# eth-cscs/conflux

Hardware: AMD Instinct MI355X
Metric: fp64_lu_tflops (higher is better)
Workload: dtype f64; 1 GPU; conflux LU N=16384 v=512 grid 1x1x1 (BASELINE cfg for 1 GPU); N=16384, v=512, grid=1x1x1

## Files before the change

conflux_amd/__init__.py:

```python
import ctypes
import os

_HERE = os.path.dirname(os.path.abspath(__file__))
_LIB_PATH = os.path.join(_HERE, "libconflux_lu.so")

UID_BYTES = 128


class ConfluxLuError(RuntimeError):
    pass


def _load():
    if not os.path.exists(_LIB_PATH):
        raise ConfluxLuError(
            f"HIP engine not built: {_LIB_PATH} missing. "
            "Run `make -C conflux_amd` (or __graft_entry__.build()). "
            "The product has no CPU fallback.")
    lib = ctypes.CDLL(_LIB_PATH)
    lib.conflux_lu_create.argtypes = [ctypes.c_int] * 7 + [
        ctypes.c_char_p, ctypes.POINTER(ctypes.c_void_p)]
    lib.conflux_lu_make_uid.argtypes = [ctypes.c_char_p]
    lib.conflux_lu_init_matrix.argtypes = [ctypes.c_void_p, ctypes.c_uint64]
    lib.conflux_lu_init_matrix_spd.argtypes = [ctypes.c_void_p, ctypes.c_uint64]
    lib.conflux_chol_factor.argtypes = [ctypes.c_void_p,
                                        ctypes.POINTER(ctypes.c_double)]
    lib.conflux_lu_set_matrix_local.argtypes = [ctypes.c_void_p, ctypes.c_void_p]
    lib.conflux_lu_set_matrix_sim.argtypes = [ctypes.c_void_p, ctypes.c_int,
                                              ctypes.c_void_p]
    lib.conflux_lu_store_factors.argtypes = [ctypes.c_void_p, ctypes.c_int]
    lib.conflux_lu_set_pivoting.argtypes = [ctypes.c_void_p, ctypes.c_int]
    lib.conflux_lu_factor.argtypes = [ctypes.c_void_p,
                                      ctypes.POINTER(ctypes.c_double)]
    lib.conflux_lu_get_factors.argtypes = [ctypes.c_void_p, ctypes.c_void_p,
                                           ctypes.c_void_p]
    lib.conflux_lu_get_factors_sim.argtypes = [ctypes.c_void_p, ctypes.c_int,
                                               ctypes.c_void_p, ctypes.c_void_p]
    lib.conflux_lu_dims.argtypes = [ctypes.c_void_p] + [
        ctypes.POINTER(ctypes.c_int)] * 6
    lib.conflux_lu_kernel_stats.argtypes = [
        ctypes.c_void_p, ctypes.c_int, ctypes.POINTER(ctypes.c_double),
        ctypes.POINTER(ctypes.c_long), ctypes.POINTER(ctypes.c_double)]
    lib.conflux_lu_validate.argtypes = [ctypes.c_void_p,
                                        ctypes.POINTER(ctypes.c_double)]
    lib.conflux_chol_validate.argtypes = [ctypes.c_void_p,
                                          ctypes.POINTER(ctypes.c_double)]
    lib.conflux_lu_destroy.argtypes = [ctypes.c_void_p]
    lib.conflux_lu_build_info.restype = ctypes.c_char_p
    lib.conflux_lu_debug_dgemm.argtypes = [
        ctypes.c_int, ctypes.c_longlong, ctypes.c_int, ctypes.c_void_p,
        ctypes.c_void_p, ctypes.c_void_p]
    lib.conflux_lu_debug_getrf.argtypes = [ctypes.c_int, ctypes.c_int,
                                           ctypes.c_void_p, ctypes.c_void_p]
    lib.conflux_lu_debug_set_panel_glue.argtypes = [ctypes.c_int]
    lib.conflux_lu_debug_set_panel_reg.argtypes = [ctypes.c_int]
    lib.conflux_lu_debug_set_panel_publish.argtypes = [ctypes.c_int]
    lib.conflux_lu_debug_set_panel_phase_stats.argtypes = [ctypes.c_int]
    lib.conflux_lu_debug_panel_phase_stats.argtypes = [ctypes.c_void_p]
    lib.conflux_lu_debug_set_trsm_stripe.argtypes = [ctypes.c_int]
    lib.conflux_lu_debug_trsm_stripe_width.argtypes = []
    lib.conflux_lu_debug_trsm_ld.argtypes = [
        ctypes.c_int, ctypes.c_int, ctypes.c_int, ctypes.c_longlong,
        ctypes.c_longlong, ctypes.c_longlong, ctypes.c_void_p,
        ctypes.c_void_p]
    lib.conflux_lu_debug_dgemm_bench.argtypes = [
        ctypes.c_int, ctypes.c_longlong, ctypes.c_int, ctypes.c_int,
        ctypes.POINTER(ctypes.c_double)]
    lib.conflux_lu_debug_trsm.argtypes = [
        ctypes.c_int, ctypes.c_int, ctypes.c_longlong, ctypes.c_int,
        ctypes.c_void_p, ctypes.c_void_p]
    lib.conflux_lu_solve.argtypes = [
        ctypes.c_void_p, ctypes.c_void_p, ctypes.c_int,
        ctypes.POINTER(ctypes.c_double)]
    lib.conflux_chol_solve.argtypes = lib.conflux_lu_solve.argtypes
    lib.conflux_lu_debug_trsm_left.argtypes = [
        ctypes.c_int, ctypes.c_int, ctypes.c_int, ctypes.c_longlong,
        ctypes.c_longlong, ctypes.c_void_p, ctypes.c_void_p]
    lib.conflux_lu_debug_update_skinny.argtypes = [
        ctypes.c_int, ctypes.c_int, ctypes.c_int, ctypes.c_longlong,
        ctypes.c_void_p, ctypes.c_void_p, ctypes.c_void_p]
    lib.conflux_lu_solve_refined.argtypes = [
        ctypes.c_void_p, ctypes.c_void_p, ctypes.c_int, ctypes.c_int,
        ctypes.c_void_p, ctypes.c_void_p, ctypes.POINTER(ctypes.c_int),
        ctypes.POINTER(ctypes.c_double)]
    lib.conflux_chol_solve_refined.argtypes = \
        lib.conflux_lu_solve_refined.argtypes
    lib.conflux_lu_debug_residual_dd.argtypes = [
        ctypes.c_int, ctypes.c_int, ctypes.c_int, ctypes.c_longlong,
        ctypes.c_void_p, ctypes.c_void_p, ctypes.c_void_p, ctypes.c_void_p]
    lib.conflux_lu_debug_residual_group_width.argtypes = []
    lib.conflux_lu_debug_residual_dd_bench.argtypes = [
        ctypes.c_int, ctypes.c_int, ctypes.c_int, ctypes.c_int,
        ctypes.POINTER(ctypes.c_double), ctypes.POINTER(ctypes.c_double)]
    lib.conflux_lu_solve_trans.argtypes = lib.conflux_lu_solve.argtypes
    lib.conflux_lu_rcond.argtypes = [
        ctypes.c_void_p, ctypes.c_int, ctypes.POINTER(ctypes.c_double),
        ctypes.POINTER(ctypes.c_double), ctypes.POINTER(ctypes.c_int),
        ctypes.POINTER(ctypes.c_double)]
    lib.conflux_chol_rcond.argtypes = [
        ctypes.c_void_p, ctypes.POINTER(ctypes.c_double),
        ctypes.POINTER(ctypes.c_double), ctypes.POINTER(ctypes.c_int),
        ctypes.POINTER(ctypes.c_double)]
    lib.conflux_lu_debug_trsm_left_trans.argtypes = \
        lib.conflux_lu_debug_trsm_left.argtypes
    lib.conflux_lu_debug_update_skinny_t.argtypes = \
        lib.conflux_lu_debug_update_skinny.argtypes
    return lib


_lib = None


def lib():
    global _lib
    if _lib is None:
        _lib = _load()
    return _lib


def _chk(rc, what):
    if rc != 0:
        raise ConfluxLuError(f"{what} failed: rc={rc}")


class Engine:

    def __init__(self, N, v, Px, Py, Pz, rank=-1, world=None, uid=None):
        import numpy as np
        self.N, self.v, self.Px, self.Py, self.Pz = N, v, Px, Py, Pz
        P = Px * Py * Pz
        world = P if world is None else world
        self.world = world
        self.sim = rank < 0
        self._h = ctypes.c_void_p()
        _chk(lib().conflux_lu_create(N, v, Px, Py, Pz, rank, world, uid,
                                     ctypes.byref(self._h)), "create")
        d = [ctypes.c_int() for _ in range(6)]
        _chk(lib().conflux_lu_dims(self._h, *[ctypes.byref(x) for x in d]),
             "dims")
        self.Ml, self.Nl, self.Nt, self.nlayr, self.M, self.Npad = \
            (x.value for x in d)

    @staticmethod
    def make_uid():
        buf = ctypes.create_string_buffer(UID_BYTES)
        _chk(lib().conflux_lu_make_uid(buf), "make_uid")
        return buf.raw

    def init_matrix(self, seed=42):
        _chk(lib().conflux_lu_init_matrix(self._h, seed), "init_matrix")

    def set_matrix_global(self, A):
        import numpy as np
        assert self.sim
        v = self.v
        for pi in range(self.Px):
            for pj in range(self.Py):
                loc = np.zeros((self.Ml, self.Nl))
                for lti in range(self.Ml // v):
                    for ltj in range(self.Nl // v):
                        gti, gtj = lti * self.Px + pi, ltj * self.Py + pj
                        loc[lti * v:(lti + 1) * v, ltj * v:(ltj + 1) * v] = \
                            A[gti * v:(gti + 1) * v, gtj * v:(gtj + 1) * v]
                loc = np.ascontiguousarray(loc)
                for pk in range(self.Pz):
                    g = (pi * self.Py + pj) * self.Pz + pk
                    buf = loc if pk == 0 else None
                    _chk(lib().conflux_lu_set_matrix_sim(
                        self._h, g,
                        buf.ctypes.data_as(ctypes.c_void_p) if buf is not None
                        else None), "set_matrix_sim")

    def set_matrix_local(self, local):
        ptr = None
        if local is not None:
            import numpy as np
            local = np.ascontiguousarray(local, dtype=np.float64)
            ptr = local.ctypes.data_as(ctypes.c_void_p)
        _chk(lib().conflux_lu_set_matrix_local(self._h, ptr), "set_matrix")

    def store_factors(self, enable):
        _chk(lib().conflux_lu_store_factors(self._h, int(enable)), "store")

    def set_pivoting(self, mode):
        _chk(lib().conflux_lu_set_pivoting(self._h, int(mode)), "pivoting")

    def factor(self):
        ms = ctypes.c_double()
        _chk(lib().conflux_lu_factor(self._h, ctypes.byref(ms)), "factor")
        return ms.value

    def init_matrix_spd(self, seed=42):
        _chk(lib().conflux_lu_init_matrix_spd(self._h, seed), "init_spd")

    def factor_cholesky(self):
        ms = ctypes.c_double()
        _chk(lib().conflux_chol_factor(self._h, ctypes.byref(ms)), "chol")
        return ms.value

    def validate(self):
        r = ctypes.c_double()
        _chk(lib().conflux_lu_validate(self._h, ctypes.byref(r)), "validate")
        return r.value

    def validate_cholesky(self):
        r = ctypes.c_double()
        _chk(lib().conflux_chol_validate(self._h, ctypes.byref(r)),
             "chol_validate")
        return r.value

    def _solve(self, fn, what, B, return_ms):
        import numpy as np
        B = np.asarray(B)
        if B.ndim not in (1, 2) or B.shape[0] != self.Npad:
            raise ValueError(
                f"{what}: B must be ({self.Npad},) or ({self.Npad}, nrhs), "
                f"got {B.shape}")
        X = np.array(B, dtype=np.float64, order="C")
        nrhs = 1 if X.ndim == 1 else X.shape[1]
        ms = ctypes.c_double()
        _chk(fn(self._h, X.ctypes.data_as(ctypes.c_void_p), nrhs,
                ctypes.byref(ms)), what)
        return (X, ms.value) if return_ms else X

    def solve(self, B, return_ms=False):
        return self._solve(lib().conflux_lu_solve, "solve", B, return_ms)

    def solve_cholesky(self, B, return_ms=False):
        return self._solve(lib().conflux_chol_solve, "solve_cholesky", B,
                           return_ms)

    def solve_transposed(self, B, return_ms=False):
        return self._solve(lib().conflux_lu_solve_trans, "solve_transposed",
                           B, return_ms)

    def _rcond(self, what, call, return_info):
        rc = ctypes.c_double()
        an = ctypes.c_double()
        ns = ctypes.c_int()
        ms = ctypes.c_double()
        _chk(call(ctypes.byref(rc), ctypes.byref(an), ctypes.byref(ns),
                  ctypes.byref(ms)), what)
        if not return_info:
            return rc.value
        return rc.value, dict(anorm=an.value, nsolves=ns.value, ms=ms.value)

    def rcond(self, norm="1", return_info=False):
        if norm not in ("1", "I"):
            raise ValueError(f'rcond: norm must be "1" or "I", got {norm!r}')
        n = 0 if norm == "1" else 1
        return self._rcond(
            "rcond", lambda *a: lib().conflux_lu_rcond(self._h, n, *a),
            return_info)

    def rcond_cholesky(self, return_info=False):
        return self._rcond(
            "rcond_cholesky",
            lambda *a: lib().conflux_chol_rcond(self._h, *a), return_info)

    def _solve_refined(self, fn, what, B, max_iter, return_info):
        import numpy as np
        B = np.asarray(B)
        if B.ndim not in (1, 2) or B.shape[0] != self.Npad:
            raise ValueError(
                f"{what}: B must be ({self.Npad},) or ({self.Npad}, nrhs), "
                f"got {B.shape}")
        X = np.array(B, dtype=np.float64, order="C")
        nrhs = 1 if X.ndim == 1 else X.shape[1]
        berr = np.zeros(nrhs)
        ferr = np.zeros(nrhs)
        iters = ctypes.c_int()
        ms = ctypes.c_double()
        _chk(fn(self._h, X.ctypes.data_as(ctypes.c_void_p), nrhs,
                int(max_iter), berr.ctypes.data_as(ctypes.c_void_p),
                ferr.ctypes.data_as(ctypes.c_void_p), ctypes.byref(iters),
                ctypes.byref(ms)), what)
        if not return_info:
            return X
        return X, dict(berr=berr, ferr=ferr, iters=iters.value, ms=ms.value)

    def solve_refined(self, B, max_iter=10, return_info=False):
        return self._solve_refined(lib().conflux_lu_solve_refined,
                                   "solve_refined", B, max_iter, return_info)

    def solve_cholesky_refined(self, B, max_iter=10, return_info=False):
        return self._solve_refined(lib().conflux_chol_solve_refined,
                                   "solve_cholesky_refined", B, max_iter,
                                   return_info)

    def get_perm(self):
        import numpy as np
        perm = np.zeros(self.M, dtype=np.int32)
        _chk(lib().conflux_lu_get_factors(self._h, None,
                                          perm.ctypes.data_as(ctypes.c_void_p)),
             "get_factors")
        return perm

    def get_F_global(self):
        import numpy as np
        assert self.sim
        v = self.v
        F = np.zeros((self.Npad, self.Npad))
        loc = np.zeros((self.Ml, self.Nl))
        for pi in range(self.Px):
            for pj in range(self.Py):
                g = (pi * self.Py + pj) * self.Pz + 0
                _chk(lib().conflux_lu_get_factors_sim(
                    self._h, g, loc.ctypes.data_as(ctypes.c_void_p), None),
                    "get_factors_sim")
                for lti in range(self.Ml // v):
                    for ltj in range(self.Nl // v):
                        gti, gtj = lti * self.Px + pi, ltj * self.Py + pj
                        F[gti * v:(gti + 1) * v, gtj * v:(gtj + 1) * v] = \
                            loc[lti * v:(lti + 1) * v, ltj * v:(ltj + 1) * v]
        return F

    def get_F_local(self):
        import numpy as np
        F = np.zeros((self.Ml, self.Nl))
        _chk(lib().conflux_lu_get_factors(self._h,
                                          F.ctypes.data_as(ctypes.c_void_p),
                                          None), "get_factors")
        return F

    def kernel_stats(self):
        out = {}
        names = {0: "dgemm_trailing", 1: "panel_getrf", 2: "trsm", 3: "rowmove"}
        for k, name in names.items():
            s = ctypes.c_double()
            n = ctypes.c_long()
            f = ctypes.c_double()
            _chk(lib().conflux_lu_kernel_stats(self._h, k, ctypes.byref(s),
                                               ctypes.byref(n),
                                               ctypes.byref(f)), "stats")
            out[name] = dict(seconds=s.value, launches=n.value, flops=f.value)
        return out

    def close(self):
        if self._h:
            lib().conflux_lu_destroy(self._h)
            self._h = None

    def __enter__(self):
        return self

    def __exit__(self, *a):
        self.close()
```

conflux_amd/csrc/engine.cpp:

```cpp
#include <hip/hip_runtime.h>
#include <rccl/rccl.h>

#include <algorithm>
#include <chrono>
#include <cmath>
#include <cstdio>
#include <cstdlib>
#include <cstring>
#include <functional>
#include <numeric>
#include <string>
#include <set>
#include <vector>

#include "../../include/conflux_lu.h"
#include "kernels.hpp"
#include "norm1est.hpp"

#define HIPCHK(x)                                                       \
    do {                                                                \
        hipError_t e_ = (x);                                            \
        if (e_ != hipSuccess) {                                         \
            std::fprintf(stderr, "[conflux_lu] HIP error %s at %s:%d\n", \
                         hipGetErrorString(e_), __FILE__, __LINE__);    \
            return CONFLUX_LU_EHIP;                                     \
        }                                                               \
    } while (0)

#define NCCLCHK(x)                                                       \
    do {                                                                 \
        ncclResult_t e_ = (x);                                           \
        if (e_ != ncclSuccess) {                                         \
            std::fprintf(stderr, "[conflux_lu] RCCL error %s at %s:%d\n", \
                         ncclGetErrorString(e_), __FILE__, __LINE__);    \
            return CONFLUX_LU_ECOMM;                                     \
        }                                                                \
    } while (0)

namespace {

struct RankState {
    int pi = 0, pj = 0, pk = 0, grank = 0;
    double *A11 = nullptr;
    double *A11in = nullptr;
    double *A10 = nullptr;
    double *A01 = nullptr;
    double *A10Rcv = nullptr;
    double *A01Rcv = nullptr;
    double *A10Rcv2 = nullptr;
    double *A01Rcv2 = nullptr;
    double *A00 = nullptr;
    double *cand = nullptr;
    double *panel = nullptr;
    double *cm = nullptr;
    double *A01pack = nullptr;
    double *rowtmp = nullptr;
    double *redtmp = nullptr;
    double *slabs = nullptr;
    double *Fres = nullptr;
    double *A10hist = nullptr;
    double *triws = nullptr;
    int *d_ipiv = nullptr;
    int *d_swap = nullptr;
    int *d_idx = nullptr;
    int *d_gri = nullptr;
    int *d_gpivots = nullptr;
    int *d_perm = nullptr;
    void *sync = nullptr;
    std::vector<int> gri;
    std::vector<int> igri;
    int *h_idx = nullptr;
    int fnp = 0, nact = 0;
};

struct TimeCat {
    double seconds = 0;
    long launches = 0;
    double flops = 0;
};

struct EvPair {
    hipEvent_t a, b;
    int cat;
    double flops;
};

struct Ctx {
    int N = 0, v = 0, Px = 1, Py = 1, Pz = 1;
    int M = 0, Ml = 0, Nl = 0, Nt = 0, Mt = 0, nlayr = 0, tA11x = 0, tA11y = 0;
    int world = 1, rank = 0;
    bool sim = false;
    bool input_dirty = true;
    bool store_factors = true;
    int factored_kind = 0;
    double anorm_inf = -1;
    double anorm_one = -1;
    int pivoting = 1;
    bool have_comm = false;
    ncclComm_t comm{};
    ncclComm_t pcomm{};
    bool have_pcomm = false;
    hipStream_t stream{};
    hipStream_t panel_stream{};
    hipStream_t trsm_stream{};
    hipEvent_t ev_pc{};
    hipEvent_t ev_t3{};
    hipEvent_t ev_t5{};
    hipEvent_t ev_t5a{};
    std::vector<RankState> rs;
    std::vector<int> pivotInds;
    unsigned epoch = 1;
    std::vector<EvPair> evs;
    size_t evs_used = 0;
    TimeCat cats[4];
    std::string err;
};

inline int grank_of(const Ctx &c, int pi, int pj, int pk) {
    return (pi * c.Py + pj) * c.Pz + pk;
}

inline int64_t i64(int a) { return (int64_t)a; }

int alloc_rank(Ctx &c, RankState &r, int pi, int pj, int pk) {
    r.pi = pi;
    r.pj = pj;
    r.pk = pk;
    r.grank = grank_of(c, pi, pj, pk);
    const int64_t Ml = c.Ml, Nl = c.Nl, v = c.v;
    const int64_t prows = std::max(i64(2 * c.v), Ml);
    HIPCHK(hipMalloc(&r.A11, Ml * Nl * 8));
    HIPCHK(hipMalloc(&r.A10, Ml * v * 8));
    HIPCHK(hipMalloc(&r.A01, v * Nl * 8));
    HIPCHK(hipMalloc(&r.A10Rcv, Ml * i64(c.nlayr) * 8));
    HIPCHK(hipMalloc(&r.A01Rcv, i64(c.nlayr) * Nl * 8));
    HIPCHK(hipMalloc(&r.A00, v * v * 8));
    HIPCHK(hipMalloc(&r.cand, i64(2 * c.v) * (v + 1) * 8));
    HIPCHK(hipMalloc(&r.panel, prows * v * 8));
    HIPCHK(hipMalloc(&r.A01pack, v * Nl * 8));
    HIPCHK(hipMalloc(&r.rowtmp, v * Nl * 8));
    HIPCHK(hipMalloc(&r.redtmp, i64(std::max(1, c.Pz - 1)) * Ml * v * 8));
    HIPCHK(hipMalloc(&r.slabs, Ml * v * 8));
    HIPCHK(hipMalloc(&r.d_ipiv, (v + 8) * 4));
    HIPCHK(hipMalloc(&r.d_swap, 128 * 4));
    HIPCHK(hipMalloc(&r.d_idx, 4 * v * 4));
    HIPCHK(hipMalloc(&r.d_gri, Ml * 4));
    HIPCHK(hipMalloc(&r.d_gpivots, v * 4));
    HIPCHK(hipMalloc(&r.d_perm, prows * 4));
    HIPCHK(hipMalloc(&r.sync, conflux_panel_sync_bytes()));
    HIPCHK(hipMemset(r.sync, 0, conflux_panel_sync_bytes()));
    HIPCHK(hipHostMalloc(&r.h_idx, size_t(2) * 4 * v * 4));
    std::memset(r.h_idx, 0, size_t(2) * 4 * v * 4);
    r.gri.resize(c.Ml);
    return 0;
}

int ensure_factor_bufs(Ctx &c, RankState &r, bool need_hist = true) {
    if (!r.Fres) HIPCHK(hipMalloc(&r.Fres, i64(c.Ml) * c.Nl * 8));
    if (need_hist && !r.A10hist)
        HIPCHK(hipMalloc(&r.A10hist, i64(c.Ml) * c.Nl * 8));
    return 0;
}

void free_rank(RankState &r) {
    for (double *p : {r.A11, r.A11in, r.A10, r.A01, r.A10Rcv, r.A01Rcv,
                      r.A10Rcv2, r.A01Rcv2,
                      r.A00, r.cand, r.panel, r.cm, r.A01pack, r.rowtmp,
                      r.redtmp, r.slabs, r.Fres, r.A10hist, r.triws})
        if (p) (void)hipFree(p);
    for (int *p : {r.d_ipiv, r.d_swap, r.d_idx, r.d_gri, r.d_gpivots, r.d_perm})
        if (p) (void)hipFree(p);
    if (r.sync) (void)hipFree(r.sync);
    if (r.h_idx) (void)hipHostFree(r.h_idx);
}

int ev_begin(Ctx &c, int cat, double flops, size_t *slot) {
    if (c.evs_used >= c.evs.size()) {
        EvPair p;
        HIPCHK(hipEventCreate(&p.a));
        HIPCHK(hipEventCreate(&p.b));
        p.cat = 0;
        p.flops = 0;
        c.evs.push_back(p);
    }
    EvPair &p = c.evs[c.evs_used];
    p.cat = cat;
    p.flops = flops;
    *slot = c.evs_used++;
    HIPCHK(hipEventRecord(p.a, c.stream));
    return 0;
}
int ev_end(Ctx &c, size_t slot) {
    HIPCHK(hipEventRecord(c.evs[slot].b, c.stream));
    return 0;
}

void nanscan(Ctx &c, const char *tag, int k, const double *p, int64_t nelem) {
    static int on = -1;
    if (on < 0) {
        const char *e = getenv("CONFLUX_NANCHECK");
        on = e ? atoi(e) : 0;
    }
    if (!on || !p || nelem <= 0) return;
    (void)hipStreamSynchronize(c.stream);
    const int64_t ns = std::min<int64_t>(nelem, 1 << 20);
    std::vector<double> s(ns);
    (void)hipMemcpy(s.data(), p, (ns / 2) * 8, hipMemcpyDeviceToHost);
    (void)hipMemcpy(s.data() + ns / 2, p + nelem - (ns - ns / 2),
                    (ns - ns / 2) * 8, hipMemcpyDeviceToHost);
    long bad = 0, zeros = 0;
    double mn = 1e300, mx = 0;
    for (double x : s) {
        if (!std::isfinite(x)) {
            ++bad;
            continue;
        }
        const double a = std::fabs(x);
        if (a == 0) ++zeros;
        if (a > mx) mx = a;
        if (a < mn) mn = a;
    }
    std::fprintf(stderr,
                 "[nanscan] k=%d %-12s bad=%ld/%lld zeros=%ld min=%.3e "
                 "max=%.3e\n",
                 k, tag, bad, (long long)ns, zeros, mn, mx);
}

int g_panel_glue = -1;
int panel_glue_mode() {
    if (g_panel_glue < 0) {
        const char *e = getenv("CONFLUX_PANEL_GLUE");
        g_panel_glue = e ? (atoi(e) != 0) : 1;
    }
    return g_panel_glue;
}

unsigned long long g_panel_phase_acc[8] = {0, 0, 0, 0, 0, 0, 0, 0};
unsigned long long g_panel_phase_cols = 0;

int factor_panel(Ctx &c, RankState &r, int n, std::vector<int> &ipiv_out) {
    const int v = c.v;
    const int NB = conflux_panel_nb();
    const int nsteps = std::min(v, n);
    ipiv_out.assign(v, 0);
    size_t slot;
    if (ev_begin(c, 1, 0, &slot)) return CONFLUX_LU_EHIP;
    auto leaf = [&](int jb, bool perm = true) -> int {
        const int nb = std::min(NB, nsteps - jb);
        const int m = n - jb;
        if (launch_panel_factor(r.panel + i64(jb) * v + jb, v, m, nb, r.sync,
                                r.d_ipiv + jb, c.epoch, r.d_swap,
                                r.d_swap + 64, c.stream)) {
            c.err = "panel grid not resident";
            return CONFLUX_LU_EINTERNAL;
        }
        c.epoch += nb;
        if (perm && v > nb)
            launch_rowperm_skip(r.panel, v, r.d_swap, r.d_swap + 64, jb,
                                2 * nb, jb, nb, v - nb, r.rowtmp, c.stream);
        return 0;
    };
    static int rec_env = -1;
    if (rec_env < 0) {
        const char *e = getenv("CONFLUX_PANEL_REC");
        rec_env = e ? atoi(e) : 0;
    }
    const int nleaf = nsteps / NB;
    if (rec_env && nsteps == v && v % NB == 0 && nleaf > 1 &&
        (nleaf & (nleaf - 1)) == 0) {
        int rc2 = 0;
        std::function<void(int, int)> rec = [&](int a, int b) {
            if (rc2) return;
            if (b - a <= NB) {
                rc2 = leaf(a);
                return;
            }
            const int h = (b - a) / 2;
            rec(a, a + h);
            if (rc2) return;
            if (h == 32)
                launch_trsm_left_lower_unit32(r.panel + i64(a) * v + a, v,
                                              r.panel + i64(a) * v + a + h, v,
                                              h, b - a - h, c.stream);
            else
                launch_trsm_left_mfma(r.panel + i64(a) * v + a, v,
                                      r.panel + i64(a) * v + a + h, v, h,
                                      b - a - h, c.stream);
            if (n > a + h)
                launch_dgemm_f64(r.panel + i64(a + h) * v + a, v,
                                 r.panel + i64(a) * v + a + h, v,
                                 r.panel + i64(a + h) * v + a + h, v,
                                 n - (a + h), b - a - h, h, c.stream);
            rec(a + h, b);
        };
        rec(0, v);
        if (rc2) return rc2;
    } else {
        const int glue = panel_glue_mode();
        for (int jb = 0; jb < nsteps; jb += NB) {
            const int nb = std::min(NB, nsteps - jb);
            const int m = n - jb;
            const bool fused = glue && nb == 32 && jb + nb < v && m > nb;
            const bool fused_perm =
                glue && nb == 32 && jb + nb == v && v > nb;
            if (leaf(jb, !(fused || fused_perm))) return CONFLUX_LU_EINTERNAL;
            if (fused || fused_perm)
                launch_panel_glue_prep(
                    r.panel, v, r.d_swap, r.d_swap + 64, jb, v - nb,
                    fused ? r.panel + i64(jb) * v + jb : nullptr, v,
                    c.stream);
            if (fused) {
                launch_panel_glue_update(r.panel + i64(jb + nb) * v + jb, v,
                                         r.panel + i64(jb) * v + jb + nb, v,
                                         r.panel + i64(jb + nb) * v + jb + nb,
                                         v, m - nb, v - jb - nb, c.stream);
            } else if (jb + nb < v && m > nb) {
                launch_trsm_left_lower_unit32(r.panel + i64(jb) * v + jb, v,
                                              r.panel + i64(jb) * v + jb + nb,
                                              v, nb, v - jb - nb, c.stream);
                static int glue_cap = -1;
                if (glue_cap < 0) {
                    const char *gc = getenv("CONFLUX_GLUE_CAP");
                    glue_cap = gc ? atoi(gc) : 0;
                }
                launch_dgemm_f64(r.panel + i64(jb + nb) * v + jb, v,
                                 r.panel + i64(jb) * v + jb + nb, v,
                                 r.panel + i64(jb + nb) * v + jb + nb, v,
                                 m - nb, v - jb - nb, nb, c.stream,
                                 glue_cap);
            }
        }
    }
    if (ev_end(c, slot)) return CONFLUX_LU_EHIP;
    std::vector<int> raw(v);
    unsigned int perr = 0;
    char *d_err = (char *)r.sync + conflux_panel_err_offset();
    HIPCHK(hipMemcpyAsync(raw.data(), r.d_ipiv, nsteps * 4,
                          hipMemcpyDeviceToHost, c.stream));
    HIPCHK(hipMemcpyAsync(&perr, d_err, 4, hipMemcpyDeviceToHost, c.stream));
    HIPCHK(hipStreamSynchronize(c.stream));
    if (perr) {
        HIPCHK(hipMemsetAsync(d_err, 0, 4, c.stream));
        if (perr >= 0x10000u)
            c.err = "panel hand-off timed out in the granule payload "
                    "re-read: column code " +
                    std::to_string(perr - 0x10000u) +
                    " (1 + sub-panel column)";
        else
            c.err = "panel hand-off timed out in the key poll: column code " +
                    std::to_string(perr) + " (1 + sub-panel column)";
        return CONFLUX_LU_EINTERNAL;
    }
    if (conflux_panel_phase_stats_mode()) {
        unsigned long long ph[8];
        conflux_panel_phase_read(r.sync, ph, c.stream);
        for (int i = 0; i < 8; ++i) g_panel_phase_acc[i] += ph[i];
        g_panel_phase_cols += nsteps;
    }
    for (int jb = 0; jb < nsteps; jb += NB) {
        const int nb = std::min(NB, nsteps - jb);
        for (int s = 0; s < nb; ++s) ipiv_out[jb + s] = jb + raw[jb + s];
    }
    return 0;
}

void ipiv_to_perm(const std::vector<int> &ipiv, int n, int v,
                  std::vector<int> &perm) {
    perm.resize(std::max(2 * v, n));
    std::iota(perm.begin(), perm.end(), 0);
    for (int i = 0; i < std::min(v, n); ++i) std::swap(perm[i], perm[ipiv[i]]);
}

int g_trsm_stripe = -1;
int trsm_stripe_mode() {
    if (g_trsm_stripe < 0) {
        const char *e = getenv("CONFLUX_TRSM_STRIPE");
        g_trsm_stripe = e ? (atoi(e) != 0) : 1;
    }
    return g_trsm_stripe;
}

int stripe_ws(RankState &r, int v, int which, double **ws) {
    const int64_t n = conflux_trsm_stripe_ws_doubles(v);
    if (!r.triws) HIPCHK(hipMalloc(&r.triws, 2 * n * 8));
    *ws = r.triws + which * n;
    return 0;
}

int fused_trsm_right(RankState &r, double *X, int64_t ldx, int v, int64_t M,
                     int trans, hipStream_t s) {
    if (trsm_stripe_mode() && conflux_trsm_stripe_fits(v)) {
        double *ws;
        if (stripe_ws(r, v, 0, &ws)) return CONFLUX_LU_EHIP;
        launch_trsm_right_stripe(r.A00, v, X, ldx, v, M, trans, ws, s);
    } else
        launch_trsm_right_mfma(r.A00, v, X, ldx, v, M, trans, s);
    return 0;
}

int fused_trsm_left(RankState &r, double *X, int64_t ldx, int v, int64_t N,
                    hipStream_t s) {
    if (trsm_stripe_mode() && conflux_trsm_stripe_fits(v)) {
        double *ws;
        if (stripe_ws(r, v, 1, &ws)) return CONFLUX_LU_EHIP;
        launch_trsm_left_stripe(r.A00, v, X, ldx, v, N, ws, s);
    } else
        launch_trsm_left_mfma(r.A00, v, X, ldx, v, N, s);
    return 0;
}

int trsm_right_upper(Ctx &c, RankState &r, double *X, int64_t ldx, int M) {
    const int v = c.v, NB = conflux_panel_nb();
    size_t slot;
    if (ev_begin(c, 2, 0, &slot)) return CONFLUX_LU_EHIP;
    if (v % 32 == 0) {
        if (fused_trsm_right(r, X, ldx, v, M, 0, c.stream))
            return CONFLUX_LU_EHIP;
        return ev_end(c, slot);
    }
    for (int jb = 0; jb < v; jb += NB) {
        const int nb = std::min(NB, v - jb);
        launch_trsm_right_upper32(r.A00 + i64(jb) * v + jb, v, X + jb, ldx, nb,
                                  M, 0, c.stream);
        if (jb + nb < v)
            launch_dgemm_f64(X + jb, ldx, r.A00 + i64(jb) * v + jb + nb, v,
                             X + jb + nb, ldx, M, v - jb - nb, nb, c.stream);
    }
    return ev_end(c, slot);
}

int trsm_left_lower(Ctx &c, RankState &r, double *X, int64_t ldx, int64_t N) {
    const int v = c.v, NB = conflux_panel_nb();
    size_t slot;
    if (ev_begin(c, 2, 0, &slot)) return CONFLUX_LU_EHIP;
    if (v % 32 == 0) {
        if (fused_trsm_left(r, X, ldx, v, N, c.stream)) return CONFLUX_LU_EHIP;
        return ev_end(c, slot);
    }
    for (int jb = 0; jb < v; jb += NB) {
        const int nb = std::min(NB, v - jb);
        launch_trsm_left_lower_unit32(r.A00 + i64(jb) * v + jb, v,
                                      X + i64(jb) * ldx, ldx, nb, N, c.stream);
        if (jb + nb < v)
            launch_dgemm_f64(r.A00 + i64(jb + nb) * v + jb, v,
                             X + i64(jb) * ldx, ldx, X + i64(jb + nb) * ldx,
                             ldx, v - jb - nb, N, nb, c.stream);
    }
    return ev_end(c, slot);
}

RankState *get_rs(Ctx &c, int pi, int pj, int pk) {
    if (c.sim) return &c.rs[grank_of(c, pi, pj, pk)];
    RankState &me = c.rs[0];
    return (me.pi == pi && me.pj == pj && me.pk == pk) ? &me : nullptr;
}

int d2d(Ctx &c, double *dst, const double *src, int64_t n) {
    HIPCHK(hipMemcpyAsync(dst, src, n * 8, hipMemcpyDeviceToDevice, c.stream));
    return 0;
}

using BufOf = std::function<double *(RankState &)>;

struct ReduceItem {
    int pi, pj;
    int64_t count;
    BufOf bufof;
};

int depth_reduce(Ctx &c, ncclComm_t comm, const std::vector<ReduceItem> &items) {
    if (c.Pz == 1) return 0;
    if (c.sim) {
        for (const auto &it : items) {
            if (it.count <= 0) continue;
            RankState &root = *get_rs(c, it.pi, it.pj, 0);
            for (int pk = 1; pk < c.Pz; ++pk)
                launch_add2d(it.bufof(*get_rs(c, it.pi, it.pj, pk)), it.count,
                             it.bufof(root), it.count, 1, it.count, c.stream);
        }
        return 0;
    }
    RankState &me = c.rs[0];
    auto slot = [&](int pk) { return me.redtmp + i64(pk - 1) * c.Ml * c.v; };
    auto mine = [&](const ReduceItem &it) {
        return it.count > 0 && it.pi == me.pi && it.pj == me.pj;
    };
    NCCLCHK(ncclGroupStart());
    for (const auto &it : items) {
        if (!mine(it)) continue;
        if (me.pk != 0)
            NCCLCHK(ncclSend(it.bufof(me), it.count, ncclDouble,
                             grank_of(c, it.pi, it.pj, 0), comm, c.stream));
        else
            for (int pk = 1; pk < c.Pz; ++pk)
                NCCLCHK(ncclRecv(slot(pk), it.count, ncclDouble,
                                 grank_of(c, it.pi, it.pj, pk), comm,
                                 c.stream));
    }
    NCCLCHK(ncclGroupEnd());
    for (const auto &it : items)
        if (mine(it) && me.pk == 0)
            for (int pk = 1; pk < c.Pz; ++pk)
                launch_add2d(slot(pk), it.count, it.bufof(me), it.count, 1,
                             it.count, c.stream);
    return 0;
}

int spread_col_slabs(Ctx &c, int kcol,
                     const std::function<int(const RankState &)> &row0_of) {
    const int v = c.v, Py = c.Py, Pz = c.Pz;
    for (auto &r : c.rs) {
        const int f = row0_of(r), n = c.Ml - f;
        const int64_t cnt = i64(n) * c.nlayr;
        double *src = r.A10 + i64(f) * v;
        if (Py == 1 && Pz == 1) {
            launch_copy2d(src, v, r.A10Rcv, c.nlayr, n, v, c.stream);
            continue;
        }
        if (n <= 0) continue;
        const bool root = r.pj == kcol && r.pk == 0;
        if (c.sim) {
            if (!root) continue;
            launch_slab_pack(src, v, n, c.nlayr, Pz, r.slabs, c.stream);
            for (int pj = 0; pj < Py; ++pj)
                for (int pk = 0; pk < Pz; ++pk)
                    if (d2d(c, get_rs(c, r.pi, pj, pk)->A10Rcv,
                            r.slabs + pk * cnt, cnt))
                        return CONFLUX_LU_EHIP;
            continue;
        }
        NCCLCHK(ncclGroupStart());
        if (root) {
            launch_slab_pack(src, v, n, c.nlayr, Pz, r.slabs, c.stream);
            for (int pj = 0; pj < Py; ++pj)
                for (int pk = 0; pk < Pz; ++pk) {
                    if (pj == kcol && pk == 0) continue;
                    NCCLCHK(ncclSend(r.slabs + pk * cnt, cnt, ncclDouble,
                                     grank_of(c, r.pi, pj, pk), c.comm,
                                     c.stream));
                }
        } else {
            NCCLCHK(ncclRecv(r.A10Rcv, cnt, ncclDouble,
                             grank_of(c, r.pi, kcol, 0), c.comm, c.stream));
        }
        NCCLCHK(ncclGroupEnd());
        if (root && d2d(c, r.A10Rcv, r.slabs, cnt)) return CONFLUX_LU_EHIP;
    }
    return 0;
}

int spread_row_panel(Ctx &c, int krow, const std::function<int64_t(int)> &w_of,
                     const std::function<int64_t(int)> &off_of) {
    const int Px = c.Px, Pz = c.Pz, nl = c.nlayr;
    for (int pj = 0; pj < c.Py; ++pj) {
        const int64_t w = w_of(pj), off = off_of(pj);
        if (w <= 0) continue;
        if (c.sim) {
            RankState &root = *get_rs(c, krow, pj, 0);
            for (int pi = 0; pi < Px; ++pi)
                for (int pk = 0; pk < Pz; ++pk)
                    launch_copy2d(root.A01 + i64(pk) * nl * w, w,
                                  get_rs(c, pi, pj, pk)->A01Rcv + off, c.Nl,
                                  nl, w, c.stream);
            continue;
        }
        RankState &me = c.rs[0];
        if (me.pj != pj) continue;
        const bool root = me.pi == krow && me.pk == 0;
        NCCLCHK(ncclGroupStart());
        if (root) {
            for (int pi = 0; pi < Px; ++pi)
                for (int pk = 0; pk < Pz; ++pk) {
                    if (pi == krow && pk == 0) continue;
                    NCCLCHK(ncclSend(me.A01 + i64(pk) * nl * w, i64(nl) * w,
                                     ncclDouble, grank_of(c, pi, pj, pk),
                                     c.comm, c.stream));
                }
        } else {
            NCCLCHK(ncclRecv(me.redtmp, i64(nl) * w, ncclDouble,
                             grank_of(c, krow, pj, 0), c.comm, c.stream));
        }
        NCCLCHK(ncclGroupEnd());
        launch_copy2d(root ? me.A01 : me.redtmp, w, me.A01Rcv + off, c.Nl, nl,
                      w, c.stream);
    }
    return 0;
}

int bcast_tile(Ctx &c, const BufOf &bufof, int64_t count, int root,
               const std::vector<int> &dests) {
    if (c.sim) {
        for (int g : dests)
            if (d2d(c, bufof(c.rs[g]), bufof(c.rs[root]), count))
                return CONFLUX_LU_EHIP;
        return 0;
    }
    RankState &me = c.rs[0];
    const bool recv =
        std::find(dests.begin(), dests.end(), me.grank) != dests.end();
    if (dests.empty() || (me.grank != root && !recv)) return 0;
    NCCLCHK(ncclGroupStart());
    if (me.grank == root)
        for (int g : dests)
            NCCLCHK(ncclSend(bufof(me), count, ncclDouble, g, c.comm,
                             c.stream));
    else
        NCCLCHK(ncclRecv(bufof(me), count, ncclDouble, root, c.comm,
                         c.stream));
    NCCLCHK(ncclGroupEnd());
    return 0;
}

int timed_region(Ctx &c, double *elapsed_ms, const std::function<int()> &body) {
    auto fence = [&]() -> int {
        HIPCHK(hipStreamSynchronize(c.stream));
        if (c.have_comm) {
            static double *scratch = nullptr;
            if (!scratch) HIPCHK(hipMalloc(&scratch, 8));
            NCCLCHK(ncclAllReduce(scratch, scratch, 1, ncclDouble, ncclSum,
                                  c.comm, c.stream));
            HIPCHK(hipStreamSynchronize(c.stream));
        }
        return 0;
    };
    if (int rc = fence()) return rc;
    const auto t1 = std::chrono::high_resolution_clock::now();
    if (int rc = body()) return rc;
    if (int rc = fence()) return rc;
    const auto t2 = std::chrono::high_resolution_clock::now();
    HIPCHK(hipGetLastError());
    if (elapsed_ms)
        *elapsed_ms =
            std::chrono::duration<double, std::milli>(t2 - t1).count();
    for (size_t i = 0; i < c.evs_used; ++i) {
        float ms = 0;
        HIPCHK(hipEventElapsedTime(&ms, c.evs[i].a, c.evs[i].b));
        TimeCat &t = c.cats[c.evs[i].cat];
        t.seconds += ms * 1e-3;
        t.launches += 1;
        t.flops += c.evs[i].flops;
    }
    return 0;
}

}

namespace {

struct StepPlan {
    std::vector<int> gpivots;
    std::vector<std::vector<int>> lrows;
    std::vector<std::vector<int>> order;
};

void plan_from_gpivots(Ctx &c, StepPlan &sp) {
    sp.lrows.assign(c.Px, {});
    sp.order.assign(c.Px, {});
    for (int i = 0; i < (int)sp.gpivots.size(); ++i) {
        const int g = sp.gpivots[i];
        const int pOwn = (g / c.v) % c.Px;
        sp.lrows[pOwn].push_back(g);
        sp.order[pOwn].push_back(i);
    }
}

int phase01(Ctx &c, int k, StepPlan &sp);
int run_step(Ctx &c, int k, StepPlan &sp);

struct GapStats {
    double to_trsm = 0, gri = 0, to_evpc = 0;
    long steps = 0, evpc_steps = 0;
};
GapStats g_gap;
bool gap_stats_on() {
    static int on = -1;
    if (on < 0) {
        const char *e = getenv("CONFLUX_GAP_STATS");
        on = e ? atoi(e) != 0 : 0;
    }
    return on != 0;
}
using GapClock = std::chrono::steady_clock;
inline double gap_ms(GapClock::time_point a, GapClock::time_point b) {
    return std::chrono::duration<double, std::milli>(b - a).count();
}

int factor_loop(Ctx &c, double *elapsed_ms) {
    for (auto &r : c.rs) {
        r.fnp = 0;
        r.nact = c.Ml;
        for (int i = 0; i < c.Ml; ++i)
            r.gri[i] = (i / c.v * c.Px + r.pi) * c.v + i % c.v;
        r.igri.assign(c.M, -1);
        for (int i = 0; i < c.Ml; ++i) r.igri[r.gri[i]] = i;
        HIPCHK(hipMemcpyAsync(r.d_gri, r.gri.data(), c.Ml * 4,
                              hipMemcpyHostToDevice, c.stream));
        if (c.store_factors) {
            if (ensure_factor_bufs(c, r)) return CONFLUX_LU_EHIP;
            launch_zero2d(r.Fres, c.Nl, c.Ml, c.Nl, c.stream);
            launch_zero2d(r.A10hist, c.Nl, c.Ml, c.Nl, c.stream);
        }
    }
    c.pivotInds.assign(c.M, -1);
    c.evs_used = 0;
    for (auto &t : c.cats) t = TimeCat{};
    g_gap = GapStats{};

    int rc = timed_region(c, elapsed_ms, [&]() -> int {
        StepPlan sp;
        int rc = phase01(c, 0, sp);
        if (rc) return rc;
        for (int k = 0; k < c.Nt; ++k) {
            rc = run_step(c, k, sp);
            if (rc) return rc;
        }
        return 0;
    });
    if (rc) return rc;
    static int spin_stats = -1;
    if (spin_stats < 0) {
        const char *e = getenv("CONFLUX_SPIN_STATS");
        spin_stats = e ? atoi(e) : 0;
    }
    if (spin_stats) {
        for (auto &r : c.rs) {
            unsigned long long sp2 = 0;
            conflux_panel_spin_read(r.sync, &sp2, c.stream);
            std::fprintf(stderr, "[spinstats] rank %d spins=%llu\n",
                         r.grank, sp2);
        }
    }
    if (conflux_panel_phase_stats_mode() && g_panel_phase_cols) {
        const unsigned long long *p = g_panel_phase_acc;
        std::fprintf(stderr,
                     "[phasestats] cols=%llu cycles all blocks: wait=%llu "
                     "load=%llu update=%llu publish=%llu | block 0: wait=%llu "
                     "load=%llu update=%llu publish=%llu\n",
                     g_panel_phase_cols, p[0], p[1], p[2], p[3], p[4], p[5],
                     p[6], p[7]);
        for (auto &x : g_panel_phase_acc) x = 0;
        g_panel_phase_cols = 0;
    }
    if (gap_stats_on())
        std::fprintf(stderr,
                     "[gapstats] steps=%ld entry->trsm=%.3f ms  gri/igri=%.3f "
                     "ms  entry->ev_pc=%.3f ms (%ld steps)\n",
                     g_gap.steps, g_gap.to_trsm, g_gap.gri, g_gap.to_evpc,
                     g_gap.evpc_steps);
    return 0;
}

int phase01(Ctx &c, int k, StepPlan &sp) {
    const int v = c.v, Px = c.Px, Py = c.Py, Pz = c.Pz;
    const int64_t Nl = c.Nl;
    const int loff = (k / Py) * v;
    const int kcol = k % Py, krow = k % Px;
    const int n_rounds = Px > 1 ? (int)std::ceil(std::log2((double)Px)) : 0;

    for (auto &r : c.rs) {
        if (r.pj != kcol) continue;
        launch_copy2d(r.A11 + i64(r.fnp) * Nl + loff, Nl,
                      r.A10 + i64(r.fnp) * v, v, r.nact, v, c.stream);
    }
    {
        std::vector<ReduceItem> items;
        for (auto &r : c.rs)
            if (r.pj == kcol && (r.pk == 0 || !c.sim))
                items.push_back({r.pi, kcol, i64(r.nact) * v,
                                 [v](RankState &x) {
                                     return x.A10 + i64(x.fnp) * v;
                                 }});
        if (depth_reduce(c, c.pcomm, items)) return CONFLUX_LU_ECOMM;
    }

    sp.gpivots.assign(v, -1);
    std::vector<int> perm;
    for (auto &r : c.rs) {
        if (r.pj != kcol || r.pk != 0) continue;
        const int n = r.nact;
        launch_copy2d(r.A10 + i64(r.fnp) * v, v, r.panel, v, n, v, c.stream);
        std::vector<int> ipiv;
        if (n > 0) {
            if (factor_panel(c, r, n, ipiv)) return CONFLUX_LU_EINTERNAL;
            for (int i = 0; i < std::min(v, n); ++i)
                if (ipiv[i] < i || ipiv[i] >= n) {
                    std::vector<double> samp(i64(std::min(n, 4096)) * v);
                    (void)hipMemcpy(samp.data(), r.panel, samp.size() * 8,
                                    hipMemcpyDeviceToHost);
                    long bad = 0;
                    double a0 = samp[0];
                    for (double x : samp)
                        if (!std::isfinite(x)) ++bad;
                    c.err = "panel ipiv out of range: k=" +
                            std::to_string(k) + " i=" + std::to_string(i) +
                            " ipiv=" + std::to_string(ipiv[i]) +
                            " n=" + std::to_string(n) +
                            " nonfinite=" + std::to_string(bad) + "/" +
                            std::to_string(samp.size()) +
                            " panel[0]=" + std::to_string(a0);
                    return CONFLUX_LU_EINTERNAL;
                }
        }
        ipiv_to_perm(ipiv, n, v, perm);
        if (n == 0) std::iota(perm.begin(), perm.end(), 0);

        if (n_rounds == 0) {
            launch_copy2d(r.panel, v, r.A00, v, std::min(v, n), v, c.stream);
            for (int i = 0; i < v; ++i)
                sp.gpivots[i] = (perm[i] < n) ? r.gri[r.fnp + perm[i]] : 0;
            if (!c.sim && c.world > 1)
                HIPCHK(hipMemcpyAsync(r.d_gpivots, sp.gpivots.data(), v * 4,
                                      hipMemcpyHostToDevice, c.stream));
        } else {
            HIPCHK(hipMemcpyAsync(r.d_perm, perm.data(), v * 4,
                                  hipMemcpyHostToDevice, c.stream));
            const int part0 = std::min(r.pi ^ 1, Px - 1);
            const int64_t off = (part0 < r.pi) ? i64(v) * (v + 1) : 0;
            launch_pack_candidate(r.A10, v, r.d_gri, r.fnp, n, v, v, r.d_perm,
                                  r.cand + off, c.stream);
        }
    }

    for (int rd = 0; rd < n_rounds; ++rd) {
        const int64_t half = i64(v) * (v + 1);
        if (!c.sim) {
            RankState &me = c.rs[0];
            if (me.pj == kcol && me.pk == 0) {
                const int src = me.pi ^ (1 << rd);
                const int64_t soff = (src < me.pi) ? half : 0;
                const int64_t roff = half - soff;
                NCCLCHK(ncclGroupStart());
                NCCLCHK(ncclSend(me.cand + soff, half, ncclDouble,
                                 grank_of(c, src, kcol, 0), c.pcomm, c.stream));
                NCCLCHK(ncclRecv(me.cand + roff, half, ncclDouble,
                                 grank_of(c, src, kcol, 0), c.pcomm, c.stream));
                NCCLCHK(ncclGroupEnd());
            }
        } else {
            for (int pi = 0; pi < Px; ++pi) {
                const int src = pi ^ (1 << rd);
                if (src < pi) continue;
                RankState &lo = *get_rs(c, pi, kcol, 0);
                RankState &hi = *get_rs(c, src, kcol, 0);
                if (d2d(c, hi.cand, lo.cand, half)) return CONFLUX_LU_EHIP;
                if (d2d(c, lo.cand + half, hi.cand + half, half))
                    return CONFLUX_LU_EHIP;
            }
        }
        for (auto &r : c.rs) {
            if (r.pj != kcol || r.pk != 0) continue;
            launch_copy2d(r.cand + 1, v + 1, r.panel, v, 2 * v, v, c.stream);
            std::vector<int> ipiv;
            if (factor_panel(c, r, 2 * v, ipiv)) return CONFLUX_LU_EINTERNAL;
            ipiv_to_perm(ipiv, 2 * v, v, perm);
            HIPCHK(hipMemcpyAsync(r.d_perm, perm.data(), v * 4,
                                  hipMemcpyHostToDevice, c.stream));
            if (rd == n_rounds - 1) {
                launch_row_gather(r.cand, v + 1, r.rowtmp, v + 1, r.d_perm, v,
                                  v + 1, c.stream);
                if (d2d(c, r.cand, r.rowtmp, i64(v) * (v + 1)))
                    return CONFLUX_LU_EHIP;
                launch_copy2d(r.panel, v, r.A00, v, v, v, c.stream);
            } else {
                const int nxt = r.pi ^ (1 << (rd + 1));
                const int64_t off = (nxt < r.pi) ? half : 0;
                launch_row_gather(r.cand, v + 1, r.rowtmp, v + 1, r.d_perm, v,
                                  v + 1, c.stream);
                if (d2d(c, r.cand + off, r.rowtmp, half)) return CONFLUX_LU_EHIP;
            }
        }
    }

    if (n_rounds > 0 || (!c.sim && c.world > 1)) {
        if (n_rounds > 0)
            for (auto &r : c.rs) {
                if (r.pj != kcol || r.pk != 0) continue;
                launch_extract_col0_int(r.cand, v + 1, v, r.d_gpivots,
                                        c.stream);
            }
        if (!c.sim) {
            RankState &me = c.rs[0];
            NCCLCHK(ncclGroupStart());
            if (me.pj == kcol && me.pk == 0 &&
                !(me.pi == krow && me.pj == kcol)) {
                NCCLCHK(ncclSend(me.A00, i64(v) * v, ncclDouble,
                                 grank_of(c, krow, me.pi, 0), c.pcomm,
                                 c.stream));
            }
            if (me.pi == krow && me.pk == 0 &&
                !(me.pj == kcol)) {
                NCCLCHK(ncclRecv(me.A00, i64(v) * v, ncclDouble,
                                 grank_of(c, me.pj, kcol, 0), c.pcomm,
                                 c.stream));
            }
            if (me.pj == kcol && me.pk == 0) {
                for (int pj = 0; pj < Py; ++pj)
                    for (int pk = 0; pk < Pz; ++pk) {
                        if (pj == kcol && pk == 0) continue;
                        NCCLCHK(ncclSend(me.d_gpivots, v, ncclInt32,
                                         grank_of(c, me.pi, pj, pk), c.pcomm,
                                         c.stream));
                    }
            } else {
                NCCLCHK(ncclRecv(me.d_gpivots, v, ncclInt32,
                                 grank_of(c, me.pi, kcol, 0), c.pcomm,
                                 c.stream));
            }
            NCCLCHK(ncclGroupEnd());
            HIPCHK(hipMemcpyAsync(sp.gpivots.data(), me.d_gpivots, v * 4,
                                  hipMemcpyDeviceToHost, c.stream));
            HIPCHK(hipStreamSynchronize(c.stream));
        } else {
            RankState &part = *get_rs(c, 0, kcol, 0);
            HIPCHK(hipMemcpyAsync(sp.gpivots.data(), part.d_gpivots, v * 4,
                                  hipMemcpyDeviceToHost, c.stream));
            for (int pi = 0; pi < Px; ++pi)
                for (int pj = 0; pj < Py; ++pj) {
                    RankState &dst = *get_rs(c, pi, pj, 0);
                    if (pi == krow && pj != kcol)
                        if (d2d(c, dst.A00, part.A00, i64(v) * v))
                            return CONFLUX_LU_EHIP;
                }
            HIPCHK(hipStreamSynchronize(c.stream));
        }
    }

    plan_from_gpivots(c, sp);
    std::copy_n(sp.gpivots.begin(), v, c.pivotInds.begin() + i64(k) * v);
    return 0;
}

int run_step(Ctx &c, int k, StepPlan &sp) {
    const int v = c.v, Px = c.Px, Py = c.Py, Pz = c.Pz;
    const int64_t Nl = c.Nl;
    const int loff = (k / Py) * v;
    const int kcol = k % Py, krow = k % Px;
    const int64_t wA01 = Nl - loff;
    const bool look = (k + 1 < c.Nt);
    const int ncol = (k + 1) % Py;
    const int64_t lnext = i64(v) * ((k + 1) / Py);
    const bool gap_on = gap_stats_on();
    GapClock::time_point gap_t0;
    if (gap_on) gap_t0 = GapClock::now();

    for (auto &r : c.rs) {
        const auto &lr = sp.lrows[r.pi];
        const auto &ord = sp.order[r.pi];
        const int cnt = (int)lr.size();
        const int f = r.fnp;
        int *const stage = r.h_idx + (k & 1) * 4 * v;
        int *const lrows_loc = stage, *const early = stage + v,
                   *const late = stage + 2 * v;
        const int wend = std::min(f + cnt, c.Ml);
        std::vector<char> in_win(std::max(wend - f, 0), 0);
        int n_early = 0, n_late = 0;
        for (int i = 0; i < cnt; ++i) {
            const int p = (lr[i] >= 0 && lr[i] < c.M) ? r.igri[lr[i]] : -1;
            if (p < 0) {
                c.err = "pivot push: global row " + std::to_string(lr[i]) +
                        " is not on rank row " + std::to_string(r.pi) +
                        " (k=" + std::to_string(k) + ")";
                return CONFLUX_LU_EINTERNAL;
            }
            lrows_loc[i] = p;
            stage[3 * v + i] = ord[i];
            if (p >= f && p < wend)
                in_win[p - f] = 1;
            else if (p >= f + cnt)
                late[n_late++] = p;
        }
        std::sort(late, late + n_late);
        n_late = (int)(std::unique(late, late + n_late) - late);
        for (int i = f; i < wend; ++i)
            if (!in_win[i - f]) early[n_early++] = i;
        if (n_early != n_late) {
            std::set<int> uniq(lr.begin(), lr.end());
            c.err = "pivot push invariant: k=" + std::to_string(k) +
                    " cnt=" + std::to_string(cnt) +
                    " uniq=" + std::to_string(uniq.size()) +
                    " early=" + std::to_string(n_early) +
                    " late=" + std::to_string(n_late) +
                    " f=" + std::to_string(f);
            return CONFLUX_LU_EINTERNAL;
        }
        if (cnt)
            HIPCHK(hipMemcpyAsync(r.d_idx, stage, size_t(4) * v * 4,
                                  hipMemcpyHostToDevice, c.stream));
        auto push = [&](double *mat, int64_t ld, int64_t cols) -> int {
            size_t slot;
            if (ev_begin(c, 3, 0, &slot)) return CONFLUX_LU_EHIP;
            launch_row_gather(mat, ld, r.rowtmp, cols, r.d_idx, cnt, cols,
                              c.stream);
            launch_row_move(mat, ld, mat, ld, r.d_idx + v, r.d_idx + 2 * v,
                            n_early, cols, c.stream);
            launch_copy2d(r.rowtmp, cols, mat + i64(f) * ld, ld, cnt, cols,
                          c.stream);
            return ev_end(c, slot);
        };
        if (push(r.A11, Nl, Nl)) return CONFLUX_LU_EHIP;
        if (push(r.A10, v, v)) return CONFLUX_LU_EHIP;
        if (c.store_factors && push(r.A10hist, Nl, Nl)) return CONFLUX_LU_EHIP;
        {
            GapClock::time_point gri_t0;
            if (gap_on) gri_t0 = GapClock::now();
            std::vector<int> tmp(cnt);
            for (int i = 0; i < cnt; ++i) tmp[i] = r.gri[lrows_loc[i]];
            for (int i = 0; i < n_late; ++i) {
                r.gri[late[i]] = r.gri[early[i]];
                r.igri[r.gri[late[i]]] = late[i];
            }
            for (int i = 0; i < cnt; ++i) {
                r.gri[f + i] = tmp[i];
                r.igri[tmp[i]] = f + i;
            }
            if (Px > 1 && cnt) {
                const int hi = n_late ? late[n_late - 1] + 1 : f + cnt;
                HIPCHK(hipMemcpyAsync(r.d_gri + f, r.gri.data() + f,
                                      size_t(hi - f) * 4,
                                      hipMemcpyHostToDevice, c.stream));
            }
            if (gap_on) g_gap.gri += gap_ms(gri_t0, GapClock::now());
        }
        r.fnp += cnt;
        r.nact -= cnt;
        launch_copy2d(r.A11 + i64(f) * Nl + loff, Nl, r.A01pack, wA01, cnt,
                      wA01, c.stream);
    }
    {
        std::vector<ReduceItem> items;
        for (int pi = 0; pi < Px; ++pi)
            for (int pj = 0; pj < Py; ++pj)
                items.push_back({pi, pj, i64(sp.lrows[pi].size()) * wA01,
                                 [](RankState &x) { return x.A01pack; }});
        if (depth_reduce(c, c.comm, items)) return CONFLUX_LU_ECOMM;
    }

    if (!c.sim) {
        RankState &me = c.rs[0];
        if (me.pk == 0) {
            NCCLCHK(ncclGroupStart());
            if (me.pi != krow) {
                const int cnt = (int)sp.lrows[me.pi].size();
                if (cnt)
                    NCCLCHK(ncclSend(me.A01pack, i64(cnt) * wA01, ncclDouble,
                                     grank_of(c, krow, me.pj, 0), c.comm,
                                     c.stream));
            } else {
                int64_t off = 0;
                for (int pi = 0; pi < Px; ++pi) {
                    if (pi == krow) continue;
                    const int cnt = (int)sp.lrows[pi].size();
                    if (cnt)
                        NCCLCHK(ncclRecv(me.redtmp + off, i64(cnt) * wA01,
                                         ncclDouble, grank_of(c, pi, me.pj, 0),
                                         c.comm, c.stream));
                    off += i64(cnt) * wA01;
                }
            }
            NCCLCHK(ncclGroupEnd());
            if (me.pi == krow) {
                const int cnt_own = (int)sp.lrows[krow].size();
                if (cnt_own) {
                    HIPCHK(hipMemcpyAsync(me.d_idx + 3 * v,
                                          sp.order[krow].data(), cnt_own * 4,
                                          hipMemcpyHostToDevice, c.stream));
                    launch_row_scatter(me.A01pack, wA01, me.A01, wA01,
                                       me.d_idx + 3 * v, cnt_own, wA01,
                                       c.stream);
                }
                int64_t off = 0;
                for (int pi = 0; pi < Px; ++pi) {
                    if (pi == krow) continue;
                    const int cnt = (int)sp.lrows[pi].size();
                    if (cnt) {
                        HIPCHK(hipMemcpyAsync(me.d_idx, sp.order[pi].data(),
                                              cnt * 4, hipMemcpyHostToDevice,
                                              c.stream));
                        launch_row_scatter(me.redtmp + off, wA01, me.A01, wA01,
                                           me.d_idx, cnt, wA01, c.stream);
                    }
                    off += i64(cnt) * wA01;
                }
            }
        }
    } else {
        for (int pj = 0; pj < Py; ++pj) {
            RankState &dst = *get_rs(c, krow, pj, 0);
            for (int pi = 0; pi < Px; ++pi) {
                RankState &src = *get_rs(c, pi, pj, 0);
                const int cnt = (int)sp.lrows[pi].size();
                if (!cnt) continue;
                HIPCHK(hipMemcpyAsync(dst.d_idx, sp.order[pi].data(), cnt * 4,
                                      hipMemcpyHostToDevice, c.stream));
                launch_row_scatter(src.A01pack, wA01, dst.A01, wA01, dst.d_idx,
                                   cnt, wA01, c.stream);
            }
        }
    }

    if (c.store_factors && k > 0) {
        const int ltik = k / Px;
        for (int pj = 0; pj < Py; ++pj) {
            const int64_t histcols =
                i64(v) * (pj < kcol ? k / Py + 1 : k / Py);
            if (histcols == 0) continue;
            for (int pi = 0; pi < Px; ++pi) {
                const int cnt = (int)sp.lrows[pi].size();
                if (!cnt) continue;
                RankState *src = get_rs(c, pi, pj, 0);
                RankState *dst = get_rs(c, krow, pj, 0);
                if (c.sim) {
                    HIPCHK(hipMemcpyAsync(dst->d_idx + 2 * v,
                                          sp.order[pi].data(), cnt * 4,
                                          hipMemcpyHostToDevice, c.stream));
                    launch_row_scatter(
                        src->A10hist + i64(src->fnp - cnt) * Nl, Nl,
                        dst->Fres + i64(ltik) * v * Nl, Nl, dst->d_idx + 2 * v,
                        cnt, histcols, c.stream);
                } else {
                    RankState &me = c.rs[0];
                    if (src && src->grank == me.grank && dst &&
                        dst->grank == me.grank) {
                        HIPCHK(hipMemcpyAsync(me.d_idx + 2 * v,
                                              sp.order[pi].data(), cnt * 4,
                                              hipMemcpyHostToDevice, c.stream));
                        launch_row_scatter(me.A10hist + i64(me.fnp - cnt) * Nl,
                                           Nl, me.Fres + i64(ltik) * v * Nl,
                                           Nl, me.d_idx + 2 * v, cnt, histcols,
                                           c.stream);
                    } else if (src && src->grank == me.grank) {
                        launch_copy2d(me.A10hist + i64(me.fnp - cnt) * Nl, Nl,
                                      me.rowtmp, histcols, cnt, histcols,
                                      c.stream);
                        NCCLCHK(ncclSend(me.rowtmp, i64(cnt) * histcols,
                                         ncclDouble,
                                         grank_of(c, krow, pj, 0), c.comm,
                                         c.stream));
                    } else if (dst && dst->grank == me.grank) {
                        NCCLCHK(ncclRecv(me.rowtmp, i64(cnt) * histcols,
                                         ncclDouble, grank_of(c, pi, pj, 0),
                                         c.comm, c.stream));
                        HIPCHK(hipMemcpyAsync(me.d_idx + 2 * v,
                                              sp.order[pi].data(), cnt * 4,
                                              hipMemcpyHostToDevice, c.stream));
                        launch_row_scatter(me.rowtmp, histcols,
                                           me.Fres + i64(ltik) * v * Nl, Nl,
                                           me.d_idx + 2 * v, cnt, histcols,
                                           c.stream);
                    }
                }
            }
        }
    }

    static int split_env = -1;
    if (split_env < 0) {
        const char *se = getenv("CONFLUX_SPLIT_TRSM");
        split_env = se ? atoi(se) : 1;
    }
    const bool split_trsm = !c.sim && c.trsm_stream && split_env;
    static int slice_env = -1;
    if (slice_env < 0) {
        const char *se2 = getenv("CONFLUX_SLICE_TRSM");
        slice_env = se2 ? atoi(se2) : 1;
    }
    const char *lk_slice = getenv("CONFLUX_LOOKAHEAD");
    const bool slice_first =
        split_trsm && slice_env && Pz == 1 && Px == 1 && look &&
        c.panel_stream && (lk_slice ? atoi(lk_slice) != 0 : true);
    auto store_u = [&](RankState &r) {
        if (!c.store_factors) return;
        double *Frow = r.Fres + i64(k / Px) * v * Nl;
        const int64_t ustart = i64(v) * (r.pj < kcol ? k / Py + 1 : k / Py);
        if (Nl - ustart > 0)
            launch_copy2d(r.A01 + (ustart - loff), wA01, Frow + ustart, Nl, v,
                          Nl - ustart, c.stream);
        if (r.pj == kcol)
            launch_copy2d(r.A00, v, Frow + loff, Nl, v, v, c.stream);
    };
    if (gap_on) {
        g_gap.to_trsm += gap_ms(gap_t0, GapClock::now());
        ++g_gap.steps;
    }
    if (split_trsm) {
        HIPCHK(hipEventRecord(c.ev_t3, c.stream));
        HIPCHK(hipStreamWaitEvent(c.trsm_stream, c.ev_t3, 0));
        hipStream_t saved = c.stream;
        c.stream = c.trsm_stream;
        for (auto &r : c.rs) {
            if (r.pi != krow || r.pk != 0) continue;
            if (slice_first) {
                const int64_t s0 = lnext - loff;
                if (trsm_left_lower(c, r, r.A01 + s0, wA01, v))
                    return CONFLUX_LU_EINTERNAL;
                HIPCHK(hipEventRecord(c.ev_t5a, c.stream));
                if (s0 > 0 && trsm_left_lower(c, r, r.A01, wA01, s0))
                    return CONFLUX_LU_EINTERNAL;
                if (wA01 - s0 - v > 0 &&
                    trsm_left_lower(c, r, r.A01 + s0 + v, wA01,
                                    wA01 - s0 - v))
                    return CONFLUX_LU_EINTERNAL;
            } else if (trsm_left_lower(c, r, r.A01, wA01, wA01))
                return CONFLUX_LU_EINTERNAL;
            store_u(r);
        }
        HIPCHK(hipEventRecord(c.ev_t5, c.stream));
        c.stream = saved;
    }

    for (auto &r : c.rs)
        nanscan(c, "A11.postpush", k, r.A11, i64(c.Ml) * Nl);
    for (auto &r : c.rs) {
        if (r.pj != kcol || r.pk != 0) continue;
        nanscan(c, "A10.pre", k, r.A10 + i64(r.fnp) * v, i64(r.nact) * v);
        nanscan(c, "A00", k, r.A00, i64(v) * v);
        if (trsm_right_upper(c, r, r.A10 + i64(r.fnp) * v, v, r.nact))
            return CONFLUX_LU_EINTERNAL;
        nanscan(c, "A10.post", k, r.A10 + i64(r.fnp) * v, i64(r.nact) * v);
        if (c.store_factors)
            launch_copy2d(r.A10 + i64(r.fnp) * v, v,
                          r.A10hist + i64(r.fnp) * Nl + loff, Nl, r.nact, v,
                          c.stream);
    }
    if (int rc = spread_col_slabs(
            c, kcol, [](const RankState &r) { return r.fnp; }))
        return rc;

    if (!split_trsm) {
        for (auto &r : c.rs) {
            if (r.pi != krow || r.pk != 0) continue;
            if (trsm_left_lower(c, r, r.A01, wA01, wA01))
                return CONFLUX_LU_EINTERNAL;
            store_u(r);
        }
    } else if (!slice_first) {
        HIPCHK(hipStreamWaitEvent(c.stream, c.ev_t5, 0));
    }
    if (Pz == 1 && Px == 1) {
        RankState &r = c.rs[0];
        if (c.sim)
            for (auto &x : c.rs)
                launch_copy2d(x.A01, wA01, x.A01Rcv, Nl, c.nlayr, wA01,
                              c.stream);
        else if (slice_first) {
            HIPCHK(hipStreamWaitEvent(c.stream, c.ev_t5a, 0));
            const int64_t s0 = lnext - loff;
            launch_copy2d(r.A01 + s0, wA01, r.A01Rcv + s0, Nl, c.nlayr, v,
                          c.stream);
        } else
            launch_copy2d(r.A01, wA01, r.A01Rcv, Nl, c.nlayr, wA01, c.stream);
    } else if (int rc = spread_row_panel(
                   c, krow, [&](int) { return wA01; },
                   [](int) { return int64_t(0); }))
        return rc;

    auto gemm_piece = [&](RankState &r, int64_t col0, int64_t ncols,
                          int cap) -> int {
        if (r.nact <= 0 || ncols <= 0) return 0;
        const double fl = 2.0 * r.nact * (double)ncols * c.nlayr;
        size_t slot;
        if (ev_begin(c, 0, fl, &slot)) return CONFLUX_LU_EHIP;
        launch_dgemm_f64(r.A10Rcv, c.nlayr, r.A01Rcv + (col0 - loff), Nl,
                         r.A11 + i64(r.fnp) * Nl + col0, Nl, r.nact, ncols,
                         c.nlayr, c.stream, cap);
        return ev_end(c, slot) ? CONFLUX_LU_EHIP : 0;
    };
    const char *lk = getenv("CONFLUX_LOOKAHEAD");
    bool async_look = look && !c.sim && c.panel_stream &&
                      (lk ? atoi(lk) != 0 : true);
    int gcap = 0;
    if (async_look) {
        static int env_cap = -1;
        if (env_cap < 0) {
            const char *e = getenv("CONFLUX_GEMM_CAP");
            env_cap = e ? atoi(e) : 432;
        }
        int panel_rows = 0;
        for (auto &r : c.rs)
            if (r.pj == ncol && r.pk == 0)
                panel_rows = std::max(panel_rows, r.nact);
        if (panel_rows > 0) {
            gcap = env_cap;
            const int nblocks = (panel_rows + conflux_panel_rpb() - 1) /
                                conflux_panel_rpb();
            const int bpc = conflux_panel_blocks_per_cu();
            const int free_cus = 256 - (gcap + 1) / 2;
            if ((nblocks + bpc - 1) / bpc > free_cus) {
                async_look = false;
                gcap = 0;
            }
        }
    }
    for (auto &r : c.rs) {
        nanscan(c, "A10Rcv", k, r.A10Rcv, i64(r.nact) * c.nlayr);
        nanscan(c, "A01Rcv", k, r.A01Rcv, i64(c.nlayr - 1) * Nl + (Nl - loff));
    }
    if (look)
        for (auto &r : c.rs)
            if (r.pj == ncol)
                if (gemm_piece(r, lnext, v, 0)) return CONFLUX_LU_EHIP;
    if (look)
        for (auto &r : c.rs)
            if (r.pj == ncol)
                nanscan(c, "A11.a-cols", k,
                        r.A11 + i64(r.fnp) * Nl + lnext, i64(r.nact) * Nl);
    if (look && !c.sim && c.panel_stream) {
        HIPCHK(hipEventRecord(c.ev_pc, c.stream));
        if (gap_on) {
            g_gap.to_evpc += gap_ms(gap_t0, GapClock::now());
            ++g_gap.evpc_steps;
        }
    }
    if (slice_first) {
        RankState &r = c.rs[0];
        HIPCHK(hipStreamWaitEvent(c.stream, c.ev_t5, 0));
        const int64_t s0 = lnext - loff;
        if (s0 > 0)
            launch_copy2d(r.A01, wA01, r.A01Rcv, Nl, c.nlayr, s0, c.stream);
        if (wA01 - s0 - v > 0)
            launch_copy2d(r.A01 + s0 + v, wA01, r.A01Rcv + s0 + v, Nl,
                          c.nlayr, wA01 - s0 - v, c.stream);
    }
    for (auto &r : c.rs) {
        if (look && r.pj == ncol) {
            if (gemm_piece(r, loff, lnext - loff, gcap)) return CONFLUX_LU_EHIP;
            if (gemm_piece(r, lnext + v, Nl - (lnext + v), gcap))
                return CONFLUX_LU_EHIP;
        } else {
            if (gemm_piece(r, loff, wA01, gcap)) return CONFLUX_LU_EHIP;
        }
    }
    if (look) {
        hipStream_t saved = c.stream;
        if (async_look) {
            HIPCHK(hipStreamWaitEvent(c.panel_stream, c.ev_pc, 0));
            c.stream = c.panel_stream;
        }
        StepPlan nsp;
        int rc = phase01(c, k + 1, nsp);
        c.stream = saved;
        if (rc) return rc;
        sp = std::move(nsp);
    }
    return 0;
}


inline int ntiles_lt(const Ctx &c, int pi, int t) {
    return (t <= pi) ? 0 : (t - pi + c.Px - 1) / c.Px;
}

std::vector<ReduceItem> static_col_items(const Ctx &c, int k) {
    std::vector<ReduceItem> items;
    for (int pi = 0; pi < c.Px; ++pi) {
        const int v = c.v, f = v * ntiles_lt(c, pi, k);
        items.push_back({pi, k % c.Py, i64(c.Ml - f) * v,
                         [f, v](RankState &x) { return x.A10 + i64(f) * v; }});
    }
    return items;
}

int potrf_tile(Ctx &c, double *T, int64_t ld) {
    const int v = c.v, NB = conflux_panel_nb();
    size_t slot;
    if (ev_begin(c, 1, 0, &slot)) return CONFLUX_LU_EHIP;
    for (int jb = 0; jb < v; jb += NB) {
        const int nb = std::min(NB, v - jb);
        launch_potrf32(T + i64(jb) * ld + jb, ld, nb, c.stream);
        if (jb + nb < v) {
            launch_trsm_right_upper32(T + i64(jb) * ld + jb, ld,
                                      T + i64(jb + nb) * ld + jb, ld, nb,
                                      v - jb - nb, 1, c.stream);
            launch_dgemm_f64_nt(T + i64(jb + nb) * ld + jb, ld,
                                T + i64(jb + nb) * ld + jb, ld,
                                T + i64(jb + nb) * ld + jb + nb, ld,
                                v - jb - nb, v - jb - nb, nb, c.stream);
        }
    }
    return ev_end(c, slot);
}

int trsm_right_lowT(Ctx &c, RankState &r, double *X, int64_t ldx, int M) {
    const int v = c.v, NB = conflux_panel_nb();
    size_t slot;
    if (ev_begin(c, 2, 0, &slot)) return CONFLUX_LU_EHIP;
    if (v % 32 == 0) {
        if (fused_trsm_right(r, X, ldx, v, M, 1, c.stream))
            return CONFLUX_LU_EHIP;
        return ev_end(c, slot);
    }
    for (int jb = 0; jb < v; jb += NB) {
        const int nb = std::min(NB, v - jb);
        launch_trsm_right_upper32(r.A00 + i64(jb) * v + jb, v, X + jb, ldx, nb,
                                  M, 1, c.stream);
        if (jb + nb < v)
            launch_dgemm_f64_nt(X + jb, ldx, r.A00 + i64(jb + nb) * v + jb, v,
                                X + jb + nb, ldx, M, v - jb - nb, nb,
                                c.stream);
    }
    return ev_end(c, slot);
}

int chol_step(Ctx &c, int k) {
    const int v = c.v, Px = c.Px, Py = c.Py, Pz = c.Pz, Nt = c.Nt;
    const int64_t Nl = c.Nl;
    const int kcol = k % Py, krow = k % Px;
    const int loff = (k / Py) * v;
    auto fnp_of = [&](int pi) { return v * ntiles_lt(c, pi, k); };
    auto f2_of = [&](int pi) { return fnp_of(pi) + (pi == krow ? v : 0); };

    for (auto &r : c.rs) {
        if (r.pj != kcol) continue;
        const int f = fnp_of(r.pi);
        launch_copy2d(r.A11 + i64(f) * Nl + loff, Nl, r.A10 + i64(f) * v, v,
                      c.Ml - f, v, c.stream);
    }
    if (depth_reduce(c, c.comm, static_col_items(c, k))) return CONFLUX_LU_ECOMM;

    {
        RankState *own = get_rs(c, krow, kcol, 0);
        if (own) {
            const int fd = fnp_of(krow);
            if (potrf_tile(c, own->A10 + i64(fd) * v, v))
                return CONFLUX_LU_EINTERNAL;
            launch_copy2d(own->A10 + i64(fd) * v, v, own->A00, v, v, v,
                          c.stream);
        }
        std::vector<int> dests;
        for (int pi = 0; pi < Px; ++pi)
            if (pi != krow) dests.push_back(grank_of(c, pi, kcol, 0));
        if (int rc = bcast_tile(c, [](RankState &x) { return x.A00; },
                                i64(v) * v, grank_of(c, krow, kcol, 0), dests))
            return rc;
    }

    for (auto &r : c.rs) {
        if (r.pj != kcol || r.pk != 0) continue;
        const int f2 = f2_of(r.pi);
        const int n2 = c.Ml - f2;
        if (n2 > 0 &&
            trsm_right_lowT(c, r, r.A10 + i64(f2) * v, v, n2))
            return CONFLUX_LU_EINTERNAL;
        if (c.store_factors) {
            if (n2 > 0)
                launch_copy2d(r.A10 + i64(f2) * v, v,
                              r.Fres + i64(f2) * Nl + loff, Nl, n2, v,
                              c.stream);
            if (r.pi == krow)
                launch_copy2d(r.A00, v, r.Fres + i64(fnp_of(krow)) * Nl + loff,
                              Nl, v, v, c.stream);
        }
    }

    if (int rc = spread_col_slabs(
            c, kcol, [&](const RankState &r) { return f2_of(r.pi); }))
        return rc;

    for (int j = k + 1; j < Nt; ++j) {
        const int rpi = j % Px, dpj = j % Py;
        const int f2r = f2_of(rpi);
        const int rowoff = ntiles_lt(c, rpi, j) * v - f2r;
        const int ltj = j / Py;
        RankState *root = get_rs(c, rpi, kcol, 0);
        if (c.sim) {
            for (int pi = 0; pi < Px; ++pi)
                for (int pk = 0; pk < Pz; ++pk) {
                    RankState &d = *get_rs(c, pi, dpj, pk);
                    const int n2 = c.Ml - f2r;
                    const double *srcslab = (Py == 1 && Pz == 1)
                        ? root->A10Rcv + i64(rowoff) * c.nlayr
                        : root->slabs + (i64(pk) * n2 + rowoff) * c.nlayr;
                    if (d2d(c, d.A01Rcv + i64(ltj) * v * c.nlayr, srcslab,
                            i64(v) * c.nlayr))
                        return CONFLUX_LU_EHIP;
                }
        } else {
            RankState &me = c.rs[0];
            const bool is_root = root && root->grank == me.grank;
            const bool is_dst = (me.pj == dpj);
            const int n2 = c.Ml - f2r;
            if (is_root) {
                const double *base = (Py == 1 && Pz == 1) ? me.A10Rcv : me.slabs;
                for (int pi = 0; pi < Px; ++pi)
                    for (int pk = 0; pk < Pz; ++pk) {
                        const double *srcslab = (Py == 1 && Pz == 1)
                            ? base + i64(rowoff) * c.nlayr
                            : base + (i64(pk) * n2 + rowoff) * c.nlayr;
                        if (pi == me.pi && dpj == me.pj && pk == me.pk) {
                            if (d2d(c, me.A01Rcv + i64(ltj) * v * c.nlayr,
                                    srcslab, i64(v) * c.nlayr))
                                return CONFLUX_LU_EHIP;
                        } else {
                            NCCLCHK(ncclGroupStart());
                            NCCLCHK(ncclSend(srcslab, i64(v) * c.nlayr,
                                             ncclDouble,
                                             grank_of(c, pi, dpj, pk), c.comm,
                                             c.stream));
                            NCCLCHK(ncclGroupEnd());
                        }
                    }
            } else if (is_dst) {
                NCCLCHK(ncclGroupStart());
                NCCLCHK(ncclRecv(me.A01Rcv + i64(ltj) * v * c.nlayr,
                                 i64(v) * c.nlayr, ncclDouble,
                                 grank_of(c, rpi, kcol, 0), c.comm, c.stream));
                NCCLCHK(ncclGroupEnd());
            }
        }
    }

    static int rect_env = -1;
    if (rect_env < 0) {
        const char *e = getenv("CONFLUX_CHOL_RECT");
        rect_env = e ? atoi(e) : 1;
    }
    for (auto &r : c.rs) {
        const int f2 = f2_of(r.pi);
        const int ltj0 = (r.pj <= k) ? (k - r.pj) / Py + 1 : 0;
        const int r0 = v * ntiles_lt(c, r.pi, k + 1);
        double fl = 0;
        for (int ltj = ltj0; ltj < c.tA11y; ++ltj) {
            const int gtj = ltj * Py + r.pj;
            if (gtj >= Nt) continue;
            const int M2 = c.Ml - v * ntiles_lt(c, r.pi, gtj);
            if (M2 > 0) fl += 2.0 * M2 * (double)v * c.nlayr;
        }
        const bool use_rect =
            rect_env && v % 128 == 0 && i64(c.Ml - r0) * 4 / 128 <= 512;
        if (use_rect) {
            const int M2r = c.Ml - r0;
            const int64_t N2 = Nl - i64(ltj0) * v;
            if (M2r <= 0 || N2 <= 0 || ltj0 >= c.tA11y) continue;
            size_t slot;
            if (ev_begin(c, 0, fl, &slot)) return CONFLUX_LU_EHIP;
            launch_dgemm_f64_nt_tril(
                r.A10Rcv + i64(r0 - f2) * c.nlayr, c.nlayr,
                r.A01Rcv + i64(ltj0) * v * c.nlayr, c.nlayr,
                r.A11 + i64(r0) * Nl + i64(ltj0) * v, Nl, M2r, N2, c.nlayr,
                v, r0, i64(ltj0) * v, Px, Py, r.pi, r.pj, c.stream);
            if (ev_end(c, slot)) return CONFLUX_LU_EHIP;
            continue;
        }
        for (int ltj = ltj0; ltj < c.tA11y; ++ltj) {
            const int gtj = ltj * Py + r.pj;
            if (gtj <= k || gtj >= Nt) continue;
            const int rstart = v * ntiles_lt(c, r.pi, gtj);
            const int M2 = c.Ml - rstart;
            if (M2 <= 0) continue;
            const double fl1 = 2.0 * M2 * (double)v * c.nlayr;
            size_t slot;
            if (ev_begin(c, 0, fl1, &slot)) return CONFLUX_LU_EHIP;
            launch_dgemm_f64_nt(r.A10Rcv + i64(rstart - f2) * c.nlayr, c.nlayr,
                                r.A01Rcv + i64(ltj) * v * c.nlayr, c.nlayr,
                                r.A11 + i64(rstart) * Nl + i64(ltj) * v, Nl,
                                M2, v, c.nlayr, c.stream);
            if (ev_end(c, slot)) return CONFLUX_LU_EHIP;
        }
    }
    return 0;
}

int chol_chain_1r(Ctx &c, int k, double *rcvA, double *rcvB) {
    const int v = c.v;
    const int64_t Nl = c.Nl;
    RankState &r = c.rs[0];
    const int fnp = k * v, f2 = fnp + v;
    launch_copy2d(r.A11 + i64(fnp) * Nl + i64(k) * v, Nl,
                  r.A10 + i64(fnp) * v, v, c.Ml - fnp, v, c.stream);
    if (potrf_tile(c, r.A10 + i64(fnp) * v, v)) return CONFLUX_LU_EINTERNAL;
    launch_copy2d(r.A10 + i64(fnp) * v, v, r.A00, v, v, v, c.stream);
    const int n2 = c.Ml - f2;
    if (n2 > 0 && trsm_right_lowT(c, r, r.A10 + i64(f2) * v, v, n2))
        return CONFLUX_LU_EINTERNAL;
    if (c.store_factors) {
        if (n2 > 0)
            launch_copy2d(r.A10 + i64(f2) * v, v,
                          r.Fres + i64(f2) * Nl + i64(k) * v, Nl, n2, v,
                          c.stream);
        launch_copy2d(r.A00, v, r.Fres + i64(fnp) * Nl + i64(k) * v, Nl, v,
                      v, c.stream);
    }
    if (n2 > 0) {
        launch_copy2d(r.A10 + i64(f2) * v, v, rcvA, c.nlayr, n2, v, c.stream);
        launch_copy2d(rcvA, c.nlayr, rcvB + i64(k + 1) * v * c.nlayr,
                      c.nlayr, n2, c.nlayr, c.stream);
    }
    return 0;
}

int chol_c4_1r(Ctx &c, int k, double *rcvA, double *rcvB, bool slice_only,
               bool rest_only) {
    const int v = c.v;
    const int64_t Nl = c.Nl;
    const int Nt = c.Nt;
    RankState &r = c.rs[0];
    const int f2 = (k + 1) * v;
    if (!rest_only && k + 1 < Nt) {
        const int M2 = c.Ml - f2;
        if (M2 > 0) {
            const double fl = 2.0 * M2 * (double)v * c.nlayr;
            size_t slot;
            if (ev_begin(c, 0, fl, &slot)) return CONFLUX_LU_EHIP;
            launch_dgemm_f64_nt(rcvA, c.nlayr,
                                rcvB + i64(k + 1) * v * c.nlayr, c.nlayr,
                                r.A11 + i64(f2) * Nl + f2, Nl, M2, v,
                                c.nlayr, c.stream);
            if (ev_end(c, slot)) return CONFLUX_LU_EHIP;
        }
    }
    if (slice_only || k + 2 >= Nt) return 0;
    const int r0 = (k + 2) * v;
    const int64_t c0 = i64(k + 2) * v;
    const int M2r = c.Ml - r0;
    const int64_t N2 = Nl - c0;
    if (M2r <= 0 || N2 <= 0) return 0;
    double fl = 0;
    for (int j = k + 2; j < Nt; ++j) fl += 2.0 * (c.Ml - i64(j) * v) * v * c.nlayr;
    const bool use_rect = v % 128 == 0 && i64(M2r) * 4 / 128 <= 512;
    static int dbg = -1;
    if (dbg < 0) {
        const char *e = getenv("CONFLUX_CHOL_DEBUG");
        dbg = e ? atoi(e) : 0;
    }
    if (dbg)
        std::fprintf(stderr, "[c4_1r] k=%d M2r=%d rect=%d\n", k, M2r,
                     (int)use_rect);
    size_t slot;
    if (ev_begin(c, 0, fl, &slot)) return CONFLUX_LU_EHIP;
    if (use_rect) {
        launch_dgemm_f64_nt_tril(rcvA + i64(r0 - f2) * c.nlayr, c.nlayr,
                                 rcvB + c0 * c.nlayr, c.nlayr,
                                 r.A11 + i64(r0) * Nl + c0, Nl, M2r, N2,
// ... 1078 lines not shown
        }
        ++it;
        if (!napplied) break;
        SCHK(hipMemcpyAsync(d_mask, mask.data(), (size_t)nrhs * 4,
                            hipMemcpyHostToDevice, c->stream));
        launch_axpy_masked(Xd, Dd, d_mask, N, nrhs, c->stream);
        SCHK(colmax(Xd, xmax));
        for (int j = 0; j < nrhs; ++j) {
            if (!mask[j]) continue;
            fe[j] = xmax[j] == 0 ? 0.0 : dmax[j] / xmax[j];
            if (dmax[j] <= u * xmax[j]) active[j] = 0;
        }
        ++applied_passes;
    }
    SCHK(hipEventRecord(e1, c->stream));
    SCHK(hipMemcpyAsync(B, Xd, xb, hipMemcpyDeviceToHost, c->stream));
    SCHK(hipStreamSynchronize(c->stream));
    SCHK(hipGetLastError());
    if (berr) std::copy(be.begin(), be.end(), berr);
    if (ferr) std::copy(fe.begin(), fe.end(), ferr);
    if (iters) *iters = applied_passes;
    if (elapsed_ms) {
        float ms = 0;
        SCHK(hipEventElapsedTime(&ms, e0, e1));
        *elapsed_ms = ms;
    }
#undef SCHK
    cleanup();
    return CONFLUX_LU_OK;
}

int conflux_lu_solve_refined(conflux_lu_ctx *c, double *B, int nrhs,
                             int max_iter, double *berr, double *ferr,
                             int *iters, double *elapsed_ms) {
    return solve_refined_common(c, false, B, nrhs, max_iter, berr, ferr,
                                iters, elapsed_ms);
}

int conflux_chol_solve_refined(conflux_lu_ctx *c, double *B, int nrhs,
                               int max_iter, double *berr, double *ferr,
                               int *iters, double *elapsed_ms) {
    return solve_refined_common(c, true, B, nrhs, max_iter, berr, ferr, iters,
                                elapsed_ms);
}

int conflux_lu_get_factors(conflux_lu_ctx *c, double *F_local, int *perm) {
    if (c->sim) return conflux_lu_get_factors_sim(c, 0, F_local, perm);
    RankState &r = c->rs[0];
    if (F_local) {
        if (!r.Fres) return CONFLUX_LU_EARG;
        HIPCHK(hipMemcpyAsync(F_local, r.Fres, i64(c->Ml) * c->Nl * 8,
                              hipMemcpyDeviceToHost, c->stream));
        HIPCHK(hipStreamSynchronize(c->stream));
    }
    if (perm) std::copy(c->pivotInds.begin(), c->pivotInds.end(), perm);
    return CONFLUX_LU_OK;
}

int conflux_lu_dims(conflux_lu_ctx *c, int *Ml, int *Nl, int *Nt, int *nlayr,
                    int *M_padded, int *N_padded) {
    if (Ml) *Ml = c->Ml;
    if (Nl) *Nl = c->Nl;
    if (Nt) *Nt = c->Nt;
    if (nlayr) *nlayr = c->nlayr;
    if (M_padded) *M_padded = c->M;
    if (N_padded) *N_padded = c->N;
    return CONFLUX_LU_OK;
}

int conflux_lu_kernel_stats(conflux_lu_ctx *c, int kernel, double *seconds,
                            long *launches, double *flops) {
    if (kernel < 0 || kernel > 3) return CONFLUX_LU_EARG;
    if (seconds) *seconds = c->cats[kernel].seconds;
    if (launches) *launches = c->cats[kernel].launches;
    if (flops) *flops = c->cats[kernel].flops;
    return CONFLUX_LU_OK;
}

int conflux_lu_debug_dgemm(int M, int64_t N, int K, const double *A,
                           const double *B, double *C) {
    hipStream_t s;
    HIPCHK(hipStreamCreate(&s));
    double *dA, *dB, *dC;
    HIPCHK(hipMalloc(&dA, i64(M) * K * 8));
    HIPCHK(hipMalloc(&dB, i64(K) * N * 8));
    HIPCHK(hipMalloc(&dC, i64(M) * N * 8));
    HIPCHK(hipMemcpy(dA, A, i64(M) * K * 8, hipMemcpyHostToDevice));
    HIPCHK(hipMemcpy(dB, B, i64(K) * N * 8, hipMemcpyHostToDevice));
    HIPCHK(hipMemcpy(dC, C, i64(M) * N * 8, hipMemcpyHostToDevice));
    launch_dgemm_f64(dA, K, dB, N, dC, N, M, N, K, s);
    HIPCHK(hipStreamSynchronize(s));
    HIPCHK(hipMemcpy(C, dC, i64(M) * N * 8, hipMemcpyDeviceToHost));
    (void)hipFree(dA); (void)hipFree(dB); (void)hipFree(dC);
    (void)hipStreamDestroy(s);
    return CONFLUX_LU_OK;
}

int conflux_lu_debug_dgemm_bench(int M, int64_t N, int K, int iters,
                                 double *tflops) {
    hipStream_t s;
    HIPCHK(hipStreamCreate(&s));
    double *dA, *dB, *dC;
    HIPCHK(hipMalloc(&dA, i64(M) * K * 8));
    HIPCHK(hipMalloc(&dB, i64(K) * N * 8));
    HIPCHK(hipMalloc(&dC, i64(M) * N * 8));
    launch_init_matrix(dA, M, K, K, 1, 1, 0, 0, 0, 7, s);
    launch_init_matrix(dB, K, (int)N, (int)N, 1, 1, 0, 0, 0, 8, s);
    launch_init_matrix(dC, M, (int)N, (int)N, 1, 1, 0, 0, 0, 9, s);
    launch_dgemm_f64(dA, K, dB, N, dC, N, M, N, K, s);
    hipEvent_t a, b;
    HIPCHK(hipEventCreate(&a));
    HIPCHK(hipEventCreate(&b));
    HIPCHK(hipEventRecord(a, s));
    for (int i = 0; i < iters; ++i)
        launch_dgemm_f64(dA, K, dB, N, dC, N, M, N, K, s);
    HIPCHK(hipEventRecord(b, s));
    HIPCHK(hipEventSynchronize(b));
    float ms = 0;
    HIPCHK(hipEventElapsedTime(&ms, a, b));
    *tflops = 2.0 * M * (double)N * K * iters / (ms * 1e-3) / 1e12;
    (void)hipFree(dA); (void)hipFree(dB); (void)hipFree(dC);
    (void)hipEventDestroy(a); (void)hipEventDestroy(b);
    (void)hipStreamDestroy(s);
    return CONFLUX_LU_OK;
}

int conflux_lu_debug_dgemm_nt_bench(int M, int64_t N, int K, int iters,
                                    double *tflops) {
    hipStream_t s;
    HIPCHK(hipStreamCreate(&s));
    double *dA, *dB, *dC;
    HIPCHK(hipMalloc(&dA, i64(M) * K * 8));
    HIPCHK(hipMalloc(&dB, N * K * 8));
    HIPCHK(hipMalloc(&dC, i64(M) * N * 8));
    launch_init_matrix(dA, M, K, K, 1, 1, 0, 0, 0, 7, s);
    launch_init_matrix(dB, (int)N, K, K, 1, 1, 0, 0, 0, 8, s);
    launch_init_matrix(dC, M, (int)N, (int)N, 1, 1, 0, 0, 0, 9, s);
    launch_dgemm_f64_nt(dA, K, dB, K, dC, N, M, N, K, s);
    hipEvent_t a, b;
    HIPCHK(hipEventCreate(&a));
    HIPCHK(hipEventCreate(&b));
    HIPCHK(hipEventRecord(a, s));
    for (int i = 0; i < iters; ++i)
        launch_dgemm_f64_nt(dA, K, dB, K, dC, N, M, N, K, s);
    HIPCHK(hipEventRecord(b, s));
    HIPCHK(hipEventSynchronize(b));
    float ms = 0;
    HIPCHK(hipEventElapsedTime(&ms, a, b));
    *tflops = 2.0 * M * (double)N * K * iters / (ms * 1e-3) / 1e12;
    (void)hipFree(dA); (void)hipFree(dB); (void)hipFree(dC);
    (void)hipEventDestroy(a); (void)hipEventDestroy(b);
    (void)hipStreamDestroy(s);
    return CONFLUX_LU_OK;
}

int conflux_lu_debug_rowmove_bench(int Ml, int64_t cols, int rows, int iters,
                                   double *gbps) {
    hipStream_t s;
    HIPCHK(hipStreamCreate(&s));
    double *src, *dst;
    int *idx;
    HIPCHK(hipMalloc(&src, i64(Ml) * cols * 8));
    HIPCHK(hipMalloc(&dst, i64(rows) * cols * 8));
    HIPCHK(hipMalloc(&idx, rows * 4));
    launch_init_matrix(src, Ml, (int)cols, (int)cols, 1, 1, 0, 0, 0, 11, s);
    std::vector<int> h(rows);
    for (int i = 0; i < rows; ++i)
        h[i] = (int)((i64(i) * 2654435761u) % Ml);
    HIPCHK(hipMemcpy(idx, h.data(), rows * 4, hipMemcpyHostToDevice));
    launch_row_gather(src, cols, dst, cols, idx, rows, cols, s);
    hipEvent_t a, b;
    HIPCHK(hipEventCreate(&a));
    HIPCHK(hipEventCreate(&b));
    HIPCHK(hipEventRecord(a, s));
    for (int i = 0; i < iters; ++i)
        launch_row_gather(src, cols, dst, cols, idx, rows, cols, s);
    HIPCHK(hipEventRecord(b, s));
    HIPCHK(hipEventSynchronize(b));
    float ms = 0;
    HIPCHK(hipEventElapsedTime(&ms, a, b));
    *gbps = 2.0 * rows * (double)cols * 8 * iters / (ms * 1e-3) / 1e9;
    (void)hipFree(src); (void)hipFree(dst); (void)hipFree(idx);
    (void)hipEventDestroy(a); (void)hipEventDestroy(b);
    (void)hipStreamDestroy(s);
    return CONFLUX_LU_OK;
}

int conflux_lu_debug_set_panel_glue(int mode) {
    const int prev = panel_glue_mode();
    g_panel_glue = mode != 0;
    return prev;
}

int conflux_lu_debug_set_panel_reg(int mode) {
    return conflux_panel_set_reg_mode(mode);
}

int conflux_lu_debug_set_panel_publish(int mode) {
    return conflux_panel_set_publish_mode(mode);
}

int conflux_lu_debug_set_panel_phase_stats(int mode) {
    return conflux_panel_set_phase_stats_mode(mode);
}

int conflux_lu_debug_panel_phase_stats(unsigned long long *out9) {
    if (!out9) return CONFLUX_LU_EARG;
    for (int i = 0; i < 8; ++i) {
        out9[i] = g_panel_phase_acc[i];
        g_panel_phase_acc[i] = 0;
    }
    out9[8] = g_panel_phase_cols;
    g_panel_phase_cols = 0;
    return CONFLUX_LU_OK;
}

int conflux_lu_debug_getrf(int n, int v, double *panel, int *ipiv_out) {
    Ctx c;
    c.v = v;
    HIPCHK(hipStreamCreate(&c.stream));
    RankState r;
    HIPCHK(hipMalloc(&r.panel, i64(std::max(n, 2 * v)) * v * 8));
    HIPCHK(hipMalloc(&r.d_ipiv, (v + 8) * 4));
    HIPCHK(hipMalloc(&r.d_swap, 128 * 4));
    HIPCHK(hipMalloc(&r.rowtmp, i64(64) * v * 8));
    HIPCHK(hipMalloc(&r.sync, conflux_panel_sync_bytes()));
    HIPCHK(hipMemset(r.sync, 0, conflux_panel_sync_bytes()));
    HIPCHK(hipMemcpy(r.panel, panel, i64(n) * v * 8, hipMemcpyHostToDevice));
    std::vector<int> ipiv;
    int rc = factor_panel(c, r, n, ipiv);
    if (!rc) {
        HIPCHK(hipMemcpy(panel, r.panel, i64(n) * v * 8,
                         hipMemcpyDeviceToHost));
        std::copy(ipiv.begin(), ipiv.end(), ipiv_out);
    }
    (void)hipFree(r.panel); (void)hipFree(r.d_ipiv);
    (void)hipFree(r.d_swap); (void)hipFree(r.rowtmp);
    (void)hipFree(r.sync);
    for (auto &e : c.evs) { (void)hipEventDestroy(e.a); (void)hipEventDestroy(e.b); }
    (void)hipStreamDestroy(c.stream);
    return rc;
}

int conflux_lu_debug_trsm(int side_right, int M_or_v, int64_t N_or_M,
                          int v, const double *T, double *X) {
    Ctx c;
    c.v = v;
    HIPCHK(hipStreamCreate(&c.stream));
    RankState r;
    HIPCHK(hipMalloc(&r.A00, i64(v) * v * 8));
    HIPCHK(hipMemcpy(r.A00, T, i64(v) * v * 8, hipMemcpyHostToDevice));
    double *dX;
    const int64_t xsz = side_right ? N_or_M * v : i64(v) * N_or_M;
    HIPCHK(hipMalloc(&dX, xsz * 8));
    HIPCHK(hipMemcpy(dX, X, xsz * 8, hipMemcpyHostToDevice));
    int rc = side_right ? trsm_right_upper(c, r, dX, v, (int)N_or_M)
                        : trsm_left_lower(c, r, dX, N_or_M, N_or_M);
    HIPCHK(hipStreamSynchronize(c.stream));
    if (!rc) HIPCHK(hipMemcpy(X, dX, xsz * 8, hipMemcpyDeviceToHost));
    (void)hipFree(r.A00); (void)hipFree(dX);
    if (r.triws) (void)hipFree(r.triws);
    for (auto &e : c.evs) { (void)hipEventDestroy(e.a); (void)hipEventDestroy(e.b); }
    (void)hipStreamDestroy(c.stream);
    (void)M_or_v;
    return rc;
}

int conflux_lu_debug_set_trsm_stripe(int mode) {
    const int prev = trsm_stripe_mode();
    g_trsm_stripe = mode != 0;
    return prev;
}

int conflux_lu_debug_trsm_stripe_width() { return conflux_trsm_stripe_width(); }

int conflux_lu_debug_trsm_ld(int side_right, int trans, int v, int64_t n,
                             int64_t ldx, int64_t off, const double *T,
                             double *X) {
    if (v <= 0 || n <= 0 || off < 0 || !T || !X ||
        ldx < off + (side_right ? i64(v) : n) || n > INT32_MAX)
        return CONFLUX_LU_EARG;
    Ctx c;
    c.v = v;
    HIPCHK(hipStreamCreate(&c.stream));
    RankState r;
    HIPCHK(hipMalloc(&r.A00, i64(v) * v * 8));
    HIPCHK(hipMemcpy(r.A00, T, i64(v) * v * 8, hipMemcpyHostToDevice));
    double *dX;
    const int64_t xsz = (side_right ? n : i64(v)) * ldx;
    HIPCHK(hipMalloc(&dX, xsz * 8));
    HIPCHK(hipMemcpy(dX, X, xsz * 8, hipMemcpyHostToDevice));
    int rc = !side_right ? trsm_left_lower(c, r, dX + off, ldx, n)
             : trans     ? trsm_right_lowT(c, r, dX + off, ldx, (int)n)
                         : trsm_right_upper(c, r, dX + off, ldx, (int)n);
    HIPCHK(hipStreamSynchronize(c.stream));
    if (!rc) HIPCHK(hipMemcpy(X, dX, xsz * 8, hipMemcpyDeviceToHost));
    (void)hipFree(r.A00); (void)hipFree(dX);
    if (r.triws) (void)hipFree(r.triws);
    for (auto &e : c.evs) { (void)hipEventDestroy(e.a); (void)hipEventDestroy(e.b); }
    (void)hipStreamDestroy(c.stream);
    return rc;
}

int conflux_lu_debug_trsm_left(int upper, int unit, int v, int64_t N,
                               int64_t ldt, const double *T, double *X) {
    if (v <= 0 || N <= 0 || ldt < v || !T || !X) return CONFLUX_LU_EARG;
    double *dT = nullptr, *dX = nullptr;
    auto cleanup = [&]() {
        for (double *p : {dT, dX})
            if (p) (void)hipFree(p);
    };
    hipError_t e = hipMalloc(&dT, i64(v) * ldt * 8);
    if (e == hipSuccess) e = hipMalloc(&dX, i64(v) * N * 8);
    if (e == hipSuccess)
        e = hipMemcpy(dT, T, i64(v) * ldt * 8, hipMemcpyHostToDevice);
    if (e == hipSuccess)
        e = hipMemcpy(dX, X, i64(v) * N * 8, hipMemcpyHostToDevice);
    if (e == hipSuccess) {
        launch_trsm_left_tri_mfma(dT, ldt, dX, N, v, N, upper, unit, nullptr);
        e = hipGetLastError();
    }
    if (e == hipSuccess) e = hipDeviceSynchronize();
    if (e == hipSuccess)
        e = hipMemcpy(X, dX, i64(v) * N * 8, hipMemcpyDeviceToHost);
    cleanup();
    HIPCHK(e);
    return CONFLUX_LU_OK;
}

int conflux_lu_debug_update_skinny(int M, int nrhs, int K, int64_t lda,
                                   const double *A, const double *B,
                                   double *C) {
    if (M <= 0 || nrhs <= 0 || nrhs > 16 || K <= 0 || lda < K || !A || !B ||
        !C)
        return CONFLUX_LU_EARG;
    double *dA = nullptr, *dB = nullptr, *dC = nullptr;
    auto cleanup = [&]() {
        for (double *p : {dA, dB, dC})
            if (p) (void)hipFree(p);
    };
    hipError_t e = hipMalloc(&dA, i64(M) * lda * 8);
    if (e == hipSuccess) e = hipMalloc(&dB, i64(K) * nrhs * 8);
    if (e == hipSuccess) e = hipMalloc(&dC, i64(M) * nrhs * 8);
    if (e == hipSuccess)
        e = hipMemcpy(dA, A, i64(M) * lda * 8, hipMemcpyHostToDevice);
    if (e == hipSuccess)
        e = hipMemcpy(dB, B, i64(K) * nrhs * 8, hipMemcpyHostToDevice);
    if (e == hipSuccess)
        e = hipMemcpy(dC, C, i64(M) * nrhs * 8, hipMemcpyHostToDevice);
    if (e == hipSuccess) {
        launch_update_skinny(dA, lda, dB, nrhs, dC, nrhs, M, nrhs, K, nullptr);
        e = hipGetLastError();
    }
    if (e == hipSuccess) e = hipDeviceSynchronize();
    if (e == hipSuccess)
        e = hipMemcpy(C, dC, i64(M) * nrhs * 8, hipMemcpyDeviceToHost);
    cleanup();
    HIPCHK(e);
    return CONFLUX_LU_OK;
}

int conflux_lu_debug_trsm_left_trans(int upper_stored, int unit, int v,
                                     int64_t N, int64_t ldt, const double *T,
                                     double *X) {
    if (v <= 0 || N <= 0 || ldt < v || !T || !X) return CONFLUX_LU_EARG;
    double *dT = nullptr, *dX = nullptr;
    auto cleanup = [&]() {
        for (double *p : {dT, dX})
            if (p) (void)hipFree(p);
    };
    hipError_t e = hipMalloc(&dT, i64(v) * ldt * 8);
    if (e == hipSuccess) e = hipMalloc(&dX, i64(v) * N * 8);
    if (e == hipSuccess)
        e = hipMemcpy(dT, T, i64(v) * ldt * 8, hipMemcpyHostToDevice);
    if (e == hipSuccess)
        e = hipMemcpy(dX, X, i64(v) * N * 8, hipMemcpyHostToDevice);
    if (e == hipSuccess) {
        launch_trsm_left_tri_mfma_t(dT, ldt, dX, N, v, N, upper_stored, unit,
                                    nullptr);
        e = hipGetLastError();
    }
    if (e == hipSuccess) e = hipDeviceSynchronize();
    if (e == hipSuccess)
        e = hipMemcpy(X, dX, i64(v) * N * 8, hipMemcpyDeviceToHost);
    cleanup();
    HIPCHK(e);
    return CONFLUX_LU_OK;
}

int conflux_lu_debug_update_skinny_t(int M, int nrhs, int K, int64_t lda,
                                     const double *A, const double *B,
                                     double *C) {
    if (M <= 0 || nrhs <= 0 || nrhs > 16 || K <= 0 || lda < M || !A || !B ||
        !C)
        return CONFLUX_LU_EARG;
    double *dA = nullptr, *dB = nullptr, *dC = nullptr;
    auto cleanup = [&]() {
        for (double *p : {dA, dB, dC})
            if (p) (void)hipFree(p);
    };
    hipError_t e = hipMalloc(&dA, i64(K) * lda * 8);
    if (e == hipSuccess) e = hipMalloc(&dB, i64(K) * nrhs * 8);
    if (e == hipSuccess) e = hipMalloc(&dC, i64(M) * nrhs * 8);
    if (e == hipSuccess)
        e = hipMemcpy(dA, A, i64(K) * lda * 8, hipMemcpyHostToDevice);
    if (e == hipSuccess)
        e = hipMemcpy(dB, B, i64(K) * nrhs * 8, hipMemcpyHostToDevice);
    if (e == hipSuccess)
        e = hipMemcpy(dC, C, i64(M) * nrhs * 8, hipMemcpyHostToDevice);
    if (e == hipSuccess) {
        launch_update_skinny_t(dA, lda, dB, nrhs, dC, nrhs, M, nrhs, K,
                               nullptr);
        e = hipGetLastError();
    }
    if (e == hipSuccess) e = hipDeviceSynchronize();
    if (e == hipSuccess)
        e = hipMemcpy(C, dC, i64(M) * nrhs * 8, hipMemcpyDeviceToHost);
    cleanup();
    HIPCHK(e);
    return CONFLUX_LU_OK;
}

int conflux_lu_debug_residual_dd(int M, int K, int nrhs, int64_t lda,
                                 const double *A, const double *X,
                                 const double *B, double *R) {
    if (M <= 0 || nrhs <= 0 || K <= 0 || lda < K || !A || !X || !B || !R)
        return CONFLUX_LU_EARG;
    double *dA = nullptr, *dX = nullptr, *dB = nullptr, *dR = nullptr;
    auto cleanup = [&]() {
        for (double *p : {dA, dX, dB, dR})
            if (p) (void)hipFree(p);
    };
    hipError_t e = hipMalloc(&dA, i64(M) * lda * 8);
    if (e == hipSuccess) e = hipMalloc(&dX, i64(K) * nrhs * 8);
    if (e == hipSuccess) e = hipMalloc(&dB, i64(M) * nrhs * 8);
    if (e == hipSuccess) e = hipMalloc(&dR, i64(M) * nrhs * 8);
    if (e == hipSuccess)
        e = hipMemcpy(dA, A, i64(M) * lda * 8, hipMemcpyHostToDevice);
    if (e == hipSuccess)
        e = hipMemcpy(dX, X, i64(K) * nrhs * 8, hipMemcpyHostToDevice);
    if (e == hipSuccess)
        e = hipMemcpy(dB, B, i64(M) * nrhs * 8, hipMemcpyHostToDevice);
    if (e == hipSuccess) {
        launch_residual_dd(dA, lda, dX, dB, dR, M, K, nrhs, nullptr);
        e = hipGetLastError();
    }
    if (e == hipSuccess) e = hipDeviceSynchronize();
    if (e == hipSuccess)
        e = hipMemcpy(R, dR, i64(M) * nrhs * 8, hipMemcpyDeviceToHost);
    cleanup();
    HIPCHK(e);
    return CONFLUX_LU_OK;
}

int conflux_lu_debug_residual_group_width() {
    return conflux_residual_group_width();
}

int conflux_lu_debug_residual_dd_bench(int M, int K, int nrhs, int iters,
                                       double *ms_resid, double *ms_copy) {
    if (M <= 0 || K <= 0 || nrhs <= 0 || iters <= 0 || !ms_resid || !ms_copy)
        return CONFLUX_LU_EARG;
    hipStream_t s;
    HIPCHK(hipStreamCreate(&s));
    double *dA, *dA2, *dX, *dB, *dR;
    HIPCHK(hipMalloc(&dA, i64(M) * K * 8));
    HIPCHK(hipMalloc(&dA2, i64(M) * K * 8));
    HIPCHK(hipMalloc(&dX, i64(K) * nrhs * 8));
    HIPCHK(hipMalloc(&dB, i64(M) * nrhs * 8));
    HIPCHK(hipMalloc(&dR, i64(M) * nrhs * 8));
    launch_init_matrix(dA, M, K, K, 1, 1, 0, 0, 0, 7, s);
    launch_init_matrix(dX, K, nrhs, nrhs, 1, 1, 0, 0, 0, 8, s);
    launch_init_matrix(dB, M, nrhs, nrhs, 1, 1, 0, 0, 0, 9, s);
    hipEvent_t a, b;
    HIPCHK(hipEventCreate(&a));
    HIPCHK(hipEventCreate(&b));
    float ms = 0;
    launch_residual_dd(dA, K, dX, dB, dR, M, K, nrhs, s);
    HIPCHK(hipEventRecord(a, s));
    for (int i = 0; i < iters; ++i)
        launch_residual_dd(dA, K, dX, dB, dR, M, K, nrhs, s);
    HIPCHK(hipEventRecord(b, s));
    HIPCHK(hipEventSynchronize(b));
    HIPCHK(hipEventElapsedTime(&ms, a, b));
    *ms_resid = ms / iters;
    HIPCHK(hipMemcpyAsync(dA2, dA, i64(M) * K * 8, hipMemcpyDeviceToDevice,
                          s));
    HIPCHK(hipEventRecord(a, s));
    for (int i = 0; i < iters; ++i)
        HIPCHK(hipMemcpyAsync(dA2, dA, i64(M) * K * 8,
                              hipMemcpyDeviceToDevice, s));
    HIPCHK(hipEventRecord(b, s));
    HIPCHK(hipEventSynchronize(b));
    HIPCHK(hipEventElapsedTime(&ms, a, b));
    *ms_copy = ms / iters;
    HIPCHK(hipGetLastError());
    (void)hipFree(dA); (void)hipFree(dA2); (void)hipFree(dX);
    (void)hipFree(dB); (void)hipFree(dR);
    (void)hipEventDestroy(a); (void)hipEventDestroy(b);
    (void)hipStreamDestroy(s);
    return CONFLUX_LU_OK;
}

int conflux_lu_destroy(conflux_lu_ctx *c) {
    for (auto &r : c->rs) free_rank(r);
    for (auto &e : c->evs) {
        (void)hipEventDestroy(e.a);
        (void)hipEventDestroy(e.b);
    }
    if (c->have_pcomm) (void)ncclCommDestroy(c->pcomm);
    if (c->have_comm) (void)ncclCommDestroy(c->comm);
    if (c->panel_stream) (void)hipStreamDestroy(c->panel_stream);
    if (c->trsm_stream) (void)hipStreamDestroy(c->trsm_stream);
    if (c->ev_pc) (void)hipEventDestroy(c->ev_pc);
    if (c->ev_t3) (void)hipEventDestroy(c->ev_t3);
    if (c->ev_t5) (void)hipEventDestroy(c->ev_t5);
    if (c->ev_t5a) (void)hipEventDestroy(c->ev_t5a);
    (void)hipStreamDestroy(c->stream);
    delete c;
    return CONFLUX_LU_OK;
}

}
```

conflux_amd/csrc/kernels.hip:

```cpp
#include <hip/hip_runtime.h>

#include <cstdint>
#include <cstdlib>

#include "kernels.hpp"

#define DEVFN __device__ __forceinline__

typedef double f64x4 __attribute__((ext_vector_type(4)));
typedef double f64x2 __attribute__((ext_vector_type(2)));
typedef double f64x2u __attribute__((ext_vector_type(2), aligned(8)));

namespace ck {

DEVFN uint64_t splitmix64(uint64_t z) {
    z += 0x9E3779B97F4A7C15ull;
    z ^= z >> 30;
    z *= 0xBF58476D1CE4E5B9ull;
    z ^= z >> 27;
    z *= 0x94D049BB133111EBull;
    z ^= z >> 31;
    return z;
}

// ... 2048 lines not shown
        hipLaunchKernelGGL((k_panel_factor<1, 256>), dim3(nblocks), dim3(256),
                           0, s, panel, ldp, m, nb, (PanelSync2 *)sync, ipiv,
                           epoch0, nblocks, swap_dst, swap_src, backoff);
    else
        hipLaunchKernelGGL((k_panel_factor<2, 256>), dim3(nblocks), dim3(256),
                           0, s, panel, ldp, m, nb, (PanelSync2 *)sync, ipiv,
                           epoch0, nblocks, swap_dst, swap_src, backoff);
    return 0;
}

void conflux_panel_spin_read(void *sync, unsigned long long *out,
                             hipStream_t s) {
    (void)hipMemcpyAsync(out, (char *)sync + offsetof(PanelSync2, spin_sum),
                         8, hipMemcpyDeviceToHost, s);
    (void)hipStreamSynchronize(s);
    (void)hipMemsetAsync((char *)sync + offsetof(PanelSync2, spin_sum), 0, 8,
                         s);
}

void conflux_panel_phase_read(void *sync, unsigned long long *out8,
                              hipStream_t s) {
    char *p = (char *)sync + offsetof(PanelSync2, phase);
    (void)hipMemcpyAsync(out8, p, 64, hipMemcpyDeviceToHost, s);
    (void)hipStreamSynchronize(s);
    (void)hipMemsetAsync(p, 0, 64, s);
}

int conflux_panel_sync_bytes() { return (int)sizeof(PanelSync2); }
int conflux_panel_err_offset() { return (int)offsetof(PanelSync2, err); }
int conflux_panel_nb() { return PANEL_NB; }
int conflux_panel_rpb() {
    int qr, tpb;
    panel_shape(&qr, &tpb);
    return qr * tpb;
}

void launch_trsm_left_lower_unit32(const double *L, int64_t ldl, double *X,
                                   int64_t ldx, int nb, int64_t N,
                                   hipStream_t s) {
    if (N <= 0 || nb <= 0) return;
    hipLaunchKernelGGL(k_trsm_left_lower_unit32, dim3(cdiv64(N, 256)),
                       dim3(256), 0, s, L, ldl, X, ldx, nb, N);
}

void launch_trsm_right_upper32(const double *U, int64_t ldu, double *X,
                               int64_t ldx, int nb, int64_t M, int trans,
                               hipStream_t s) {
    if (M <= 0 || nb <= 0) return;
    hipLaunchKernelGGL(k_trsm_right_upper32, dim3(cdiv64(M, 256)), dim3(256),
                       0, s, U, ldu, X, ldx, nb, M, trans);
}


#define TRM_ROWS 128
__global__ __launch_bounds__(256) void k_trsm_right_mfma(
    const double *__restrict__ U, int64_t ldu, double *__restrict__ X,
    int64_t ldx, int v, int64_t M, int trans) {
    __shared__ double sXj[TRM_ROWS][33];
    __shared__ double sXp[2][TRM_ROWS][33];
    __shared__ double sU[2][32][33];
    const int tid = threadIdx.x;
    const int lane = tid & 63, wave = tid >> 6;
    const int frow = lane & 15, fk = lane >> 4;
    const int64_t r0 = (int64_t)blockIdx.x * TRM_ROWS;
    const int rows = (int)min((int64_t)TRM_ROWS, M - r0);
    double rx[16], ru[4];
    auto load_u_regs = [&](int pb, int jb) {
#pragma unroll
        for (int i = 0; i < 4; ++i) {
            const int e = tid + i * 256;
            ru[i] = trans
                        ? U[(int64_t)(jb + (e & 31)) * ldu + pb + (e >> 5)]
                        : U[(int64_t)(pb + (e >> 5)) * ldu + jb + (e & 31)];
        }
    };
    auto load_x_regs = [&](int pb) {
#pragma unroll
        for (int i = 0; i < 16; ++i) {
            const int e = tid + i * 256;
            rx[i] = (e >> 5) < rows
                        ? X[(r0 + (e >> 5)) * ldx + pb + (e & 31)]
                        : 0.0;
        }
    };
    auto write_bufs = [&](int buf) {
#pragma unroll
        for (int i = 0; i < 16; ++i) {
            const int e = tid + i * 256;
            sXp[buf][e >> 5][e & 31] = rx[i];
        }
#pragma unroll
        for (int i = 0; i < 4; ++i) {
            const int e = tid + i * 256;
            sU[buf][e >> 5][e & 31] = ru[i];
        }
    };
    for (int jb = 0; jb < v; jb += 32) {
        __syncthreads();
        for (int i = tid; i < rows * 32; i += 256)
            sXj[i >> 5][i & 31] = X[(r0 + (i >> 5)) * ldx + jb + (i & 31)];
        int cur = 0;
        if (jb > 0) {
            load_x_regs(0);
            load_u_regs(0, jb);
            write_bufs(0);
        }
        __syncthreads();
        for (int pb = 0; pb < jb; pb += 32) {
            if (pb + 32 < jb) {
                load_x_regs(pb + 32);
                load_u_regs(pb + 32, jb);
            }
            if (wave * 32 < rows) {
#pragma unroll
                for (int rt = 0; rt < 2; ++rt) {
                    const int rbase = wave * 32 + rt * 16;
                    f64x4 acc[2] = {f64x4{0, 0, 0, 0}, f64x4{0, 0, 0, 0}};
#pragma unroll
                    for (int kk = 0; kk < 8; ++kk) {
                        const int k = kk * 4 + fk;
                        const double a = sXp[cur][rbase + frow][k];
#pragma unroll
                        for (int ct = 0; ct < 2; ++ct)
                            acc[ct] = __builtin_amdgcn_mfma_f64_16x16x4f64(
                                a, sU[cur][k][ct * 16 + frow], acc[ct], 0, 0,
                                0);
                    }
#pragma unroll
                    for (int ct = 0; ct < 2; ++ct)
#pragma unroll
                        for (int q = 0; q < 4; ++q)
                            sXj[rbase + 4 * q + fk][ct * 16 + frow] -=
                                acc[ct][q];
                }
            }
            if (pb + 32 < jb) write_bufs(cur ^ 1);
            __syncthreads();
            cur ^= 1;
        }
        for (int i = tid; i < 32 * 32; i += 256)
            sU[0][i >> 5][i & 31] =
                trans ? U[(int64_t)(jb + (i & 31)) * ldu + jb + (i >> 5)]
                      : U[(int64_t)(jb + (i >> 5)) * ldu + jb + (i & 31)];
        __syncthreads();
        if (tid < rows) {
            double x[32];
#pragma unroll
            for (int c = 0; c < 32; ++c) x[c] = sXj[tid][c];
#pragma unroll
            for (int c = 0; c < 32; ++c) {
                double acc = x[c];
#pragma unroll
                for (int i = 0; i < 32; ++i)
                    if (i < c) acc -= x[i] * sU[0][i][c];
                x[c] = acc / sU[0][c][c];
            }
#pragma unroll
            for (int c = 0; c < 32; ++c) sXj[tid][c] = x[c];
        }
        __syncthreads();
        for (int i = tid; i < rows * 32; i += 256)
            X[(r0 + (i >> 5)) * ldx + jb + (i & 31)] = sXj[i >> 5][i & 31];
    }
}

#define TRM_COLS 128
__global__ __launch_bounds__(256) void k_trsm_left_mfma(
    const double *__restrict__ L, int64_t ldl, double *__restrict__ X,
    int64_t ldx, int v, int64_t N) {
    __shared__ double sXj[32][TRM_COLS + 1];
    __shared__ double sXp[2][32][TRM_COLS + 1];
    __shared__ double sL[2][32][33];
    const int tid = threadIdx.x;
    const int lane = tid & 63, wave = tid >> 6;
    const int frow = lane & 15, fk = lane >> 4;
    const int64_t c0 = (int64_t)blockIdx.x * TRM_COLS;
    const int cols = (int)min((int64_t)TRM_COLS, N - c0);
    double rx[16], rl[4];
    auto load_l_regs = [&](int pb, int jb) {
#pragma unroll
        for (int i = 0; i < 4; ++i) {
            const int e = tid + i * 256;
            rl[i] = L[(int64_t)(jb + (e >> 5)) * ldl + pb + (e & 31)];
        }
    };
    auto load_x_regs = [&](int pb) {
#pragma unroll
        for (int i = 0; i < 16; ++i) {
            const int e = tid + i * 256;
            rx[i] = (e & (TRM_COLS - 1)) < cols
                        ? X[(int64_t)(pb + (e >> 7)) * ldx + c0 +
                            (e & (TRM_COLS - 1))]
                        : 0.0;
        }
    };
    auto write_bufs = [&](int buf) {
#pragma unroll
        for (int i = 0; i < 16; ++i) {
            const int e = tid + i * 256;
            sXp[buf][e >> 7][e & (TRM_COLS - 1)] = rx[i];
        }
#pragma unroll
        for (int i = 0; i < 4; ++i) {
            const int e = tid + i * 256;
            sL[buf][e >> 5][e & 31] = rl[i];
        }
    };
    for (int jb = 0; jb < v; jb += 32) {
        __syncthreads();
        for (int i = tid; i < 32 * TRM_COLS; i += 256)
            if ((i & (TRM_COLS - 1)) < cols)
                sXj[i >> 7][i & (TRM_COLS - 1)] =
                    X[(int64_t)(jb + (i >> 7)) * ldx + c0 +
                      (i & (TRM_COLS - 1))];
        int cur = 0;
        if (jb > 0) {
            load_x_regs(0);
            load_l_regs(0, jb);
            write_bufs(0);
        }
        __syncthreads();
        for (int pb = 0; pb < jb; pb += 32) {
            if (pb + 32 < jb) {
                load_x_regs(pb + 32);
                load_l_regs(pb + 32, jb);
            }
            if (wave * 32 < cols) {
#pragma unroll
                for (int ct = 0; ct < 2; ++ct) {
                    const int cbase = wave * 32 + ct * 16;
                    f64x4 acc[2] = {f64x4{0, 0, 0, 0}, f64x4{0, 0, 0, 0}};
#pragma unroll
                    for (int kk = 0; kk < 8; ++kk) {
                        const int k = kk * 4 + fk;
                        const double b = sXp[cur][k][cbase + frow];
#pragma unroll
                        for (int rt = 0; rt < 2; ++rt)
                            acc[rt] = __builtin_amdgcn_mfma_f64_16x16x4f64(
                                sL[cur][rt * 16 + frow][k], b, acc[rt], 0, 0,
                                0);
                    }
#pragma unroll
                    for (int rt = 0; rt < 2; ++rt)
#pragma unroll
                        for (int q = 0; q < 4; ++q)
                            sXj[rt * 16 + 4 * q + fk][cbase + frow] -=
                                acc[rt][q];
                }
            }
            if (pb + 32 < jb) write_bufs(cur ^ 1);
            __syncthreads();
            cur ^= 1;
        }
        for (int i = tid; i < 32 * 32; i += 256)
            sL[0][i >> 5][i & 31] =
                L[(int64_t)(jb + (i >> 5)) * ldl + jb + (i & 31)];
        __syncthreads();
        if (tid < cols) {
            double x[32];
#pragma unroll
            for (int r = 0; r < 32; ++r) x[r] = sXj[r][tid];
#pragma unroll
            for (int k = 0; k < 32; ++k) {
                const double xk = x[k];
#pragma unroll
                for (int r = 0; r < 32; ++r)
                    if (r > k) x[r] -= sL[0][r][k] * xk;
            }
#pragma unroll
            for (int r = 0; r < 32; ++r) sXj[r][tid] = x[r];
        }
        __syncthreads();
        for (int i = tid; i < 32 * TRM_COLS; i += 256)
            if ((i & (TRM_COLS - 1)) < cols)
                X[(int64_t)(jb + (i >> 7)) * ldx + c0 + (i & (TRM_COLS - 1))] =
                    sXj[i >> 7][i & (TRM_COLS - 1)];
    }
}

#define TRS_W 32
#define TRS_MAXP 16

__global__ __launch_bounds__(256) void k_trsm_pack_tri(
    const double *__restrict__ T, int64_t ld, double *__restrict__ P, int swap,
    int tr) {
    int j = 0;
    while ((j + 1) * (j + 2) / 2 <= (int)blockIdx.x) ++j;
    const int pb = ((int)blockIdx.x - j * (j + 1) / 2) * 32, jb = j * 32;
    const int rb = swap ? jb : pb, cb = swap ? pb : jb;
#pragma unroll
    for (int i = 0; i < 4; ++i) {
        const int e = threadIdx.x + i * 256;
        const int r = e >> 5, c = e & 31;
        P[(int64_t)blockIdx.x * 1024 + e] =
            T[(int64_t)(rb + (tr ? c : r)) * ld + cb + (tr ? r : c)];
    }
}

__device__ inline int trs_blk(int pb, int jb) {
    return ((jb >> 5) * ((jb >> 5) + 1) / 2 + (pb >> 5)) * 1024;
}

__global__ __launch_bounds__(256) void k_trsm_right_stripe(
    const double *__restrict__ U, double *__restrict__ X, int64_t ldx, int v,
    int64_t M) {
    __shared__ double sX[TRS_MAXP][TRS_W][33];
    __shared__ double sU[2][32][33];
    const int tid = threadIdx.x;
    const int lane = tid & 63, wave = tid >> 6;
    const int frow = lane & 15, fk = lane >> 4;
    const int rt = wave >> 1, ct = wave & 1;
    const int64_t r0 = (int64_t)blockIdx.x * TRS_W;
    const int rows = (int)min((int64_t)TRS_W, M - r0);
    double ru[4];
    auto load_u_regs = [&](int pb, int jb) {
#pragma unroll
        for (int i = 0; i < 4; ++i) ru[i] = U[trs_blk(pb, jb) + tid + i * 256];
    };
    auto write_u = [&](int buf) {
#pragma unroll
        for (int i = 0; i < 4; ++i) {
            const int e = tid + i * 256;
            sU[buf][e >> 5][e & 31] = ru[i];
        }
    };
    load_u_regs(0, 0);
    for (int i = tid; i < TRS_W * v; i += 256) {
        const int r = i / v, cc = i - r * v;
        sX[cc >> 5][r][cc & 31] = r < rows ? X[(r0 + r) * ldx + cc] : 0.0;
    }
    write_u(0);
    __syncthreads();
    int cur = 0;
    for (int jb = 0; jb < v; jb += 32) {
        double(*sXj)[33] = sX[jb >> 5];
        for (int pb = 0; pb < jb; pb += 32) {
            load_u_regs(pb + 32, jb);
            const double(*sXp)[33] = sX[pb >> 5];
            f64x4 acc = {0, 0, 0, 0};
#pragma unroll
            for (int kk = 0; kk < 8; ++kk) {
                const int k = kk * 4 + fk;
                acc = __builtin_amdgcn_mfma_f64_16x16x4f64(
                    sXp[rt * 16 + frow][k], sU[cur][k][ct * 16 + frow], acc, 0,
                    0, 0);
            }
#pragma unroll
            for (int q = 0; q < 4; ++q)
                sXj[rt * 16 + 4 * q + fk][ct * 16 + frow] -= acc[q];
            write_u(cur ^ 1);
            __syncthreads();
            cur ^= 1;
        }
        const bool more = jb + 32 < v;
        if (more) load_u_regs(0, jb + 32);
        if (tid < rows) {
            double x[32];
#pragma unroll
            for (int c = 0; c < 32; ++c) x[c] = sXj[tid][c];
#pragma unroll
            for (int c = 0; c < 32; ++c) {
                double acc = x[c];
#pragma unroll
                for (int i = 0; i < 32; ++i)
                    if (i < c) acc -= x[i] * sU[cur][i][c];
                x[c] = acc / sU[cur][c][c];
            }
#pragma unroll
            for (int c = 0; c < 32; ++c) sXj[tid][c] = x[c];
        }
        if (more) write_u(cur ^ 1);
        __syncthreads();
        cur ^= 1;
    }
    for (int i = tid; i < rows * v; i += 256) {
        const int r = i / v, cc = i - r * v;
        X[(r0 + r) * ldx + cc] = sX[cc >> 5][r][cc & 31];
    }
}

__global__ __launch_bounds__(256) void k_trsm_left_stripe(
    const double *__restrict__ L, double *__restrict__ X, int64_t ldx, int v,
    int64_t N) {
    __shared__ double sX[TRS_MAXP][32][TRS_W + 1];
    __shared__ double sL[2][32][33];
    const int tid = threadIdx.x;
    const int lane = tid & 63, wave = tid >> 6;
    const int frow = lane & 15, fk = lane >> 4;
    const int rt = wave >> 1, ct = wave & 1;
    const int64_t c0 = (int64_t)blockIdx.x * TRS_W;
    const int cols = (int)min((int64_t)TRS_W, N - c0);
    double rl[4];
    auto load_l_regs = [&](int pb, int jb) {
#pragma unroll
        for (int i = 0; i < 4; ++i) rl[i] = L[trs_blk(pb, jb) + tid + i * 256];
    };
    auto write_l = [&](int buf) {
#pragma unroll
        for (int i = 0; i < 4; ++i) {
            const int e = tid + i * 256;
            sL[buf][e >> 5][e & 31] = rl[i];
        }
    };
    load_l_regs(0, 0);
    for (int i = tid; i < v * TRS_W; i += 256) {
        const int r = i >> 5, cc = i & (TRS_W - 1);
        sX[r >> 5][r & 31][cc] =
            cc < cols ? X[(int64_t)r * ldx + c0 + cc] : 0.0;
    }
    write_l(0);
    __syncthreads();
    int cur = 0;
    for (int jb = 0; jb < v; jb += 32) {
        double(*sXj)[TRS_W + 1] = sX[jb >> 5];
        for (int pb = 0; pb < jb; pb += 32) {
            load_l_regs(pb + 32, jb);
            const double(*sXp)[TRS_W + 1] = sX[pb >> 5];
            f64x4 acc = {0, 0, 0, 0};
#pragma unroll
            for (int kk = 0; kk < 8; ++kk) {
                const int k = kk * 4 + fk;
                acc = __builtin_amdgcn_mfma_f64_16x16x4f64(
                    sL[cur][rt * 16 + frow][k], sXp[k][ct * 16 + frow], acc, 0,
                    0, 0);
            }
#pragma unroll
            for (int q = 0; q < 4; ++q)
                sXj[rt * 16 + 4 * q + fk][ct * 16 + frow] -= acc[q];
            write_l(cur ^ 1);
            __syncthreads();
            cur ^= 1;
        }
        const bool more = jb + 32 < v;
        if (more) load_l_regs(0, jb + 32);
        if (tid < cols) {
            double x[32];
#pragma unroll
            for (int r = 0; r < 32; ++r) x[r] = sXj[r][tid];
#pragma unroll
            for (int k = 0; k < 32; ++k) {
                const double xk = x[k];
#pragma unroll
                for (int r = 0; r < 32; ++r)
                    if (r > k) x[r] -= sL[cur][r][k] * xk;
            }
#pragma unroll
            for (int r = 0; r < 32; ++r) sXj[r][tid] = x[r];
        }
        if (more) write_l(cur ^ 1);
        __syncthreads();
        cur ^= 1;
    }
    for (int i = tid; i < v * TRS_W; i += 256) {
        const int r = i >> 5, cc = i & (TRS_W - 1);
        if (cc < cols) X[(int64_t)r * ldx + c0 + cc] = sX[r >> 5][r & 31][cc];
    }
}

int conflux_trsm_stripe_width() { return TRS_W; }
bool conflux_trsm_stripe_fits(int v) {
    return v > 0 && v % 32 == 0 && v <= 32 * TRS_MAXP;
}

int64_t conflux_trsm_stripe_ws_doubles(int v) {
    const int64_t np = v / 32;
    return np * (np + 1) / 2 * 1024;
}

void launch_trsm_right_stripe(const double *U, int64_t ldu, double *X,
                              int64_t ldx, int v, int64_t M, int trans,
                              double *ws, hipStream_t s) {
    if (M <= 0 || v <= 0) return;
    const int nblk = (int)(conflux_trsm_stripe_ws_doubles(v) / 1024);
    hipLaunchKernelGGL(k_trsm_pack_tri, dim3(nblk), dim3(256), 0, s, U, ldu, ws,
                       trans ? 1 : 0, trans ? 1 : 0);
    hipLaunchKernelGGL(k_trsm_right_stripe, dim3(cdiv64(M, TRS_W)), dim3(256),
                       0, s, ws, X, ldx, v, M);
}

void launch_trsm_left_stripe(const double *L, int64_t ldl, double *X,
                             int64_t ldx, int v, int64_t N, double *ws,
                             hipStream_t s) {
    if (N <= 0 || v <= 0) return;
    const int nblk = (int)(conflux_trsm_stripe_ws_doubles(v) / 1024);
    hipLaunchKernelGGL(k_trsm_pack_tri, dim3(nblk), dim3(256), 0, s, L, ldl, ws,
                       1, 0);
    hipLaunchKernelGGL(k_trsm_left_stripe, dim3(cdiv64(N, TRS_W)), dim3(256),
                       0, s, ws, X, ldx, v, N);
}

void launch_trsm_right_mfma(const double *U, int64_t ldu, double *X,
                            int64_t ldx, int v, int64_t M, int trans,
                            hipStream_t s) {
    if (M <= 0 || v <= 0) return;
    hipLaunchKernelGGL(k_trsm_right_mfma, dim3(cdiv64(M, TRM_ROWS)),
                       dim3(256), 0, s, U, ldu, X, ldx, v, M, trans);
}

void launch_trsm_left_mfma(const double *L, int64_t ldl, double *X,
                           int64_t ldx, int v, int64_t N, hipStream_t s) {
    if (N <= 0 || v <= 0) return;
    hipLaunchKernelGGL(k_trsm_left_mfma, dim3(cdiv64(N, TRM_COLS)), dim3(256),
                       0, s, L, ldl, X, ldx, v, N);
}

__global__ void k_tril_unit(const double *__restrict__ F, double *__restrict__ L,
                            int64_t n) {
    const int64_t stride = (int64_t)gridDim.x * blockDim.x;
    for (int64_t i = (int64_t)blockIdx.x * blockDim.x + threadIdx.x;
         i < n * n; i += stride) {
        const int64_t r = i / n, c = i % n;
        L[i] = (r > c) ? F[i] : (r == c ? 1.0 : 0.0);
    }
}

__global__ void k_tril(const double *__restrict__ F, double *__restrict__ L,
                       int64_t n) {
    const int64_t stride = (int64_t)gridDim.x * blockDim.x;
    for (int64_t i = (int64_t)blockIdx.x * blockDim.x + threadIdx.x;
         i < n * n; i += stride) {
        const int64_t r = i / n, c = i % n;
        L[i] = (r >= c) ? F[i] : 0.0;
    }
}

__global__ void k_triu(const double *__restrict__ F, double *__restrict__ U,
                       int64_t n) {
    const int64_t stride = (int64_t)gridDim.x * blockDim.x;
    for (int64_t i = (int64_t)blockIdx.x * blockDim.x + threadIdx.x;
         i < n * n; i += stride) {
        const int64_t r = i / n, c = i % n;
        U[i] = (r <= c) ? F[i] : 0.0;
    }
}

__global__ void k_frob2(const double *__restrict__ A, int64_t n,
                        double *__restrict__ out) {
    __shared__ double part[256];
    const int tid = threadIdx.x;
    double s = 0;
    for (int64_t i = (int64_t)blockIdx.x * 256 + tid; i < n;
         i += (int64_t)gridDim.x * 256)
        s += A[i] * A[i];
    part[tid] = s;
    __syncthreads();
    for (int w = 128; w > 0; w >>= 1) {
        if (tid < w) part[tid] += part[tid + w];
        __syncthreads();
    }
    if (tid == 0) (void)atomicAdd(out, part[0]);
}

void launch_tril_unit(const double *F, double *L, int64_t n, hipStream_t s) {
    hipLaunchKernelGGL(k_tril_unit, dim3(cap_grid(n * n)), dim3(256), 0, s,
                       F, L, n);
}

__global__ void k_tril_unit_rows(const double *__restrict__ F, int64_t ldf,
                                 double *__restrict__ L, int64_t ldl,
                                 int rows, int64_t row0, int64_t ncols) {
    const int64_t stride = (int64_t)gridDim.x * blockDim.x;
    for (int64_t i = (int64_t)blockIdx.x * blockDim.x + threadIdx.x;
         i < (int64_t)rows * ncols; i += stride) {
        const int64_t r = i / ncols, c = i % ncols, g = row0 + r;
        L[r * ldl + c] = (g > c) ? F[r * ldf + c] : (g == c ? 1.0 : 0.0);
    }
}

__global__ void k_triu_rows(double *__restrict__ F, int64_t ldf, int rows,
                            int64_t row0) {
    const int64_t stride = (int64_t)gridDim.x * blockDim.x;
    const int64_t w = row0 + rows;
    for (int64_t i = (int64_t)blockIdx.x * blockDim.x + threadIdx.x;
         i < (int64_t)rows * w; i += stride) {
        const int64_t r = i / w, c = i % w;
        if (c < row0 + r) F[r * ldf + c] = 0.0;
    }
}

void launch_tril_unit_rows(const double *F, int64_t ldf, double *L,
                           int64_t ldl, int rows, int64_t row0, int64_t ncols,
                           hipStream_t s) {
    if (rows <= 0 || ncols <= 0) return;
    hipLaunchKernelGGL(k_tril_unit_rows, dim3(cap_grid((int64_t)rows * ncols)),
                       dim3(256), 0, s, F, ldf, L, ldl, rows, row0, ncols);
}

void launch_triu_rows(double *F, int64_t ldf, int rows, int64_t row0,
                      hipStream_t s) {
    if (rows <= 0) return;
    hipLaunchKernelGGL(k_triu_rows,
                       dim3(cap_grid((int64_t)rows * (row0 + rows))),
                       dim3(256), 0, s, F, ldf, rows, row0);
}
__global__ void k_sym_mirror_up(double *__restrict__ A, int64_t n) {
    const int64_t stride = (int64_t)gridDim.x * blockDim.x;
    for (int64_t i = (int64_t)blockIdx.x * blockDim.x + threadIdx.x;
         i < n * n; i += stride) {
        const int64_t r = i / n, c = i % n;
        if (r < c) A[i] = A[c * n + r];
    }
}

void launch_transpose_add_lower(double *A, int64_t n, hipStream_t s) {
    hipLaunchKernelGGL(k_sym_mirror_up, dim3(cap_grid(n * n)), dim3(256),
                       0, s, A, n);
}

void launch_tril(const double *F, double *L, int64_t n, hipStream_t s) {
    hipLaunchKernelGGL(k_tril, dim3(cap_grid(n * n)), dim3(256), 0, s, F,
                       L, n);
}
void launch_triu(const double *F, double *U, int64_t n, hipStream_t s) {
    hipLaunchKernelGGL(k_triu, dim3(cap_grid(n * n)), dim3(256), 0, s, F,
                       U, n);
}
void launch_frob2(const double *A, int64_t nelem, double *out, hipStream_t s) {
    int blocks = (int)cdiv64(nelem, 256 * 16);
    if (blocks > 4096) blocks = 4096;
    if (blocks < 1) blocks = 1;
    hipLaunchKernelGGL(k_frob2, dim3(blocks), dim3(256), 0, s, A, nelem, out);
}

void launch_potrf32(double *A, int64_t lda, int nb, hipStream_t s) {
    if (nb <= 0) return;
    hipLaunchKernelGGL(k_potrf32, dim3(1), dim3(256), 0, s, A, lda, nb);
}

void launch_getrf32_nopiv(double *A, int64_t lda, int nb, hipStream_t s) {
    if (nb <= 0) return;
    hipLaunchKernelGGL(k_getrf32_nopiv, dim3(1), dim3(256), 0, s, A, lda, nb);
}

int g_dgemm_variant = -1;

static int gemm_strip_w() {
    static int w = -1;
    if (w < 0) {
        const char *e = getenv("CONFLUX_GEMM_STRIP");
        w = e ? atoi(e) : 8;
    }
    return w;
}

static int gemm_ntc() {
    static int v = -1;
    if (v < 0) {
        const char *e = getenv("CONFLUX_GEMM_NTC");
        v = e ? atoi(e) : 0;
    }
    return v;
}

void launch_dgemm_f64(const double *A, int64_t lda, const double *B,
                      int64_t ldb, double *C, int64_t ldc, int M, int64_t N,
                      int K, hipStream_t s, int maxwg) {
    if (M <= 0 || N <= 0 || K <= 0) return;
    if (g_dgemm_variant < 0) {
        const char *e = getenv("CONFLUX_GEMM_VARIANT");
        g_dgemm_variant = e ? atoi(e) : 1;
    }
    const int ntm = (int)cdiv64(M, GEMM_BM);
    const int ntn = (int)cdiv64(N, GEMM_BN);
    const int sw = gemm_strip_w();
    int nwg = ntm * ntn;
    if (maxwg > 0 && g_dgemm_variant == 1 && nwg > maxwg) nwg = maxwg;
    if (g_dgemm_variant == 3) {
        const int ntm2 = (int)cdiv64(M, 256);
        hipLaunchKernelGGL(k_dgemm_f64_bm256, dim3(ntm2 * ntn), dim3(512), 0,
                           s, A, lda, B, ldb, C, ldc, M, N, K, ntm2, ntn, sw);
        return;
    }
    if (g_dgemm_variant == 2)
        hipLaunchKernelGGL(k_dgemm_f64_glds, dim3(ntm * ntn), dim3(512), 0, s,
                           A, lda, B, ldb, C, ldc, M, N, K, ntm, ntn, sw);
    else if (g_dgemm_variant == 1)
        hipLaunchKernelGGL(k_dgemm_f64_w8, dim3(nwg), dim3(512), 0, s,
                           A, lda, B, ldb, C, ldc, M, N, K, ntm, ntn, sw,
                           gemm_ntc());
    else
        hipLaunchKernelGGL(k_dgemm_f64, dim3(ntm * ntn), dim3(GEMM_TPB), 0, s,
                           A, lda, B, ldb, C, ldc, M, N, K, ntm, ntn, sw);
}

void launch_dgemm_f64_nt(const double *A, int64_t lda, const double *B,
                         int64_t ldb, double *C, int64_t ldc, int M, int64_t N,
                         int K, hipStream_t s) {
    if (M <= 0 || N <= 0 || K <= 0) return;
    const int ntm = (int)cdiv64(M, GEMM_BM);
    const int ntn = (int)cdiv64(N, GEMM_BN);
    hipLaunchKernelGGL(k_dgemm_f64_w8_nt, dim3(ntm * ntn), dim3(512), 0, s, A,
                       lda, B, ldb, C, ldc, M, N, K, ntm, ntn, gemm_strip_w(),
                       TriMask{0, 0, 0, 0, 0, 0, 0});
}

void launch_dgemm_f64_nt_tril(const double *A, int64_t lda, const double *B,
                              int64_t ldb, double *C, int64_t ldc, int M,
                              int64_t N, int K, int v, int r0off,
                              int64_t c0off, int Px, int Py, int pi, int pj,
                              hipStream_t s) {
    if (M <= 0 || N <= 0 || K <= 0) return;
    const int ntm = (int)cdiv64(M, GEMM_BM);
    const int ntn = (int)cdiv64(N, GEMM_BN);
    hipLaunchKernelGGL(k_dgemm_f64_w8_nt, dim3(ntm * ntn), dim3(512), 0, s, A,
                       lda, B, ldb, C, ldc, M, N, K, ntm, ntn, gemm_strip_w(),
                       TriMask{v, r0off, c0off, Px, Py, pi, pj});
}

void launch_pack_candidate(const double *A10, int64_t lda, const int *gri,
                           int f, int n_src, int n_out, int v, const int *idx,
                           double *cand, hipStream_t s) {
    if (n_out <= 0) return;
    hipLaunchKernelGGL(k_pack_candidate,
                       dim3(cdiv64((int64_t)n_out * (v + 1), 256)), dim3(256),
                       0, s, A10, lda, gri, f, n_src, n_out, v, idx, cand);
}

void launch_row_move(const double *src, int64_t lds, double *dst, int64_t ldd,
                     const int *src_idx, const int *dst_idx, int n_rows,
                     int64_t cols, hipStream_t s) {
    if (n_rows <= 0 || cols <= 0) return;
    hipLaunchKernelGGL(k_row_move, dim3(cap_grid((int64_t)n_rows * cols)),
                       dim3(256), 0, s, src, lds, dst, ldd, src_idx, dst_idx,
                       n_rows, cols);
}

void launch_extract_col0_int(const double *cand, int stride, int n, int *out,
                             hipStream_t s) {
    if (n <= 0) return;
    hipLaunchKernelGGL(k_extract_col0_int, dim3(cdiv64(n, 256)), dim3(256), 0,
                       s, cand, stride, n, out);
}

void launch_slab_pack(const double *X, int64_t ldx, int n, int nlayr, int Pz,
                      double *out, hipStream_t s) {
    if (n <= 0) return;
    hipLaunchKernelGGL(k_slab_pack,
                       dim3(cdiv64((int64_t)n * nlayr * Pz, 256)), dim3(256),
                       0, s, X, ldx, n, nlayr, Pz, out);
}
```

conflux_amd/csrc/kernels.hpp:

```cpp
#pragma once
#include <hip/hip_runtime.h>

#include <cstdint>

#define CONFLUX_PANEL_MAX_BLOCKS 256

void launch_init_matrix(double *A, int Ml, int Nl, int v, int Px, int Py,
                        int pi, int pj, int zero_layer, uint64_t seed,
                        hipStream_t s);
void launch_copy2d(const double *src, int64_t lds, double *dst, int64_t ldd,
                   int rows, int64_t cols, hipStream_t s);
void launch_zero2d(double *dst, int64_t ldd, int rows, int64_t cols,
                   hipStream_t s);
void launch_add2d(const double *src, int64_t lds, double *dst, int64_t ldd,
                  int rows, int64_t cols, hipStream_t s);
void launch_row_gather(const double *src, int64_t lds, double *dst,
                       int64_t ldd, const int *idx, int n_rows, int64_t cols,
                       hipStream_t s);
void launch_row_scatter(const double *src, int64_t lds, double *dst,
                        int64_t ldd, const int *idx, int n_rows, int64_t cols,
                        hipStream_t s);
void launch_rowperm_skip(double *mat, int64_t ld, const int *dst_idx,
                         const int *src_idx, int row_base, int n_rows,
                         int64_t skip0, int64_t skipn, int64_t tot_cols,
                         double *tmp, hipStream_t s);
void launch_panel_glue_prep(double *mat, int64_t ld, const int *dst_idx,
                            const int *src_idx, int jb, int tot_cols,
                            const double *L, int64_t ldl, hipStream_t s);
void launch_panel_glue_update(const double *A, int64_t lda, const double *B,
                              int64_t ldb, double *C, int64_t ldc, int M,
                              int N, hipStream_t s);
int launch_panel_factor(double *panel, int64_t ldp, int m, int nb, void *sync,
                        int *ipiv, unsigned int epoch0, int *swap_dst,
                        int *swap_src, hipStream_t s);
int conflux_panel_sync_bytes();
int conflux_panel_err_offset();
void conflux_panel_spin_read(void *sync, unsigned long long *out,
                             hipStream_t s);
int conflux_panel_reg_mode();
int conflux_panel_publish_mode();
int conflux_panel_phase_stats_mode();
int conflux_panel_set_reg_mode(int mode);
int conflux_panel_set_publish_mode(int mode);
int conflux_panel_set_phase_stats_mode(int mode);
void conflux_panel_phase_read(void *sync, unsigned long long *out8,
                              hipStream_t s);
int conflux_panel_nb();
int conflux_panel_rpb();
int conflux_panel_blocks_per_cu();
void launch_trsm_left_lower_unit32(const double *L, int64_t ldl, double *X,
                                   int64_t ldx, int nb, int64_t N,
                                   hipStream_t s);
void launch_trsm_right_upper32(const double *U, int64_t ldu, double *X,
                               int64_t ldx, int nb, int64_t M, int trans,
                               hipStream_t s);
void launch_trsm_right_mfma(const double *U, int64_t ldu, double *X,
                            int64_t ldx, int v, int64_t M, int trans,
                            hipStream_t s);
void launch_trsm_left_mfma(const double *L, int64_t ldl, double *X,
                           int64_t ldx, int v, int64_t N, hipStream_t s);
int conflux_trsm_stripe_width();
bool conflux_trsm_stripe_fits(int v);
int64_t conflux_trsm_stripe_ws_doubles(int v);
void launch_trsm_right_stripe(const double *U, int64_t ldu, double *X,
                              int64_t ldx, int v, int64_t M, int trans,
                              double *ws, hipStream_t s);
void launch_trsm_left_stripe(const double *L, int64_t ldl, double *X,
                             int64_t ldx, int v, int64_t N, double *ws,
                             hipStream_t s);
void launch_trsm_left_tri_mfma(const double *T, int64_t ldt, double *X,
                               int64_t ldx, int v, int64_t N, int upper,
                               int unit, hipStream_t s);
void launch_update_skinny(const double *A, int64_t lda, const double *B,
                          int64_t ldb, double *C, int64_t ldc, int M, int nrhs,
                          int K, hipStream_t s);
void launch_trsm_left_tri_mfma_t(const double *T, int64_t ldt, double *X,
                                 int64_t ldx, int v, int64_t N,
                                 int upper_stored, int unit, hipStream_t s);
void launch_update_skinny_t(const double *A, int64_t lda, const double *B,
                            int64_t ldb, double *C, int64_t ldc, int M,
                            int nrhs, int K, hipStream_t s);
void launch_col_abs_sums(const double *A, int64_t lda, int M, int K,
                         double *out, hipStream_t s);
void launch_residual_dd(const double *A, int64_t lda, const double *X,
                        const double *B, double *R, int M, int K, int nrhs,
                        hipStream_t s);
int conflux_residual_group_width();
void launch_row_abs_sums(const double *A, int64_t lda, int M, int K,
                         double *out, hipStream_t s);
void launch_colmax_abs(const double *V, int64_t n, int ncols, double *out,
                       hipStream_t s);
void launch_axpy_masked(double *X, const double *D, const int *mask,
                        int64_t n, int ncols, hipStream_t s);
void launch_tril_unit(const double *F, double *L, int64_t n, hipStream_t s);
void launch_tril_unit_rows(const double *F, int64_t ldf, double *L,
                           int64_t ldl, int rows, int64_t row0, int64_t ncols,
                           hipStream_t s);
void launch_triu_rows(double *F, int64_t ldf, int rows, int64_t row0,
                      hipStream_t s);
void launch_transpose_add_lower(double *A, int64_t n, hipStream_t s);
void launch_tril(const double *F, double *L, int64_t n, hipStream_t s);
void launch_triu(const double *F, double *U, int64_t n, hipStream_t s);
void launch_frob2(const double *A, int64_t nelem, double *out, hipStream_t s);
void launch_potrf32(double *A, int64_t lda, int nb, hipStream_t s);
void launch_getrf32_nopiv(double *A, int64_t lda, int nb, hipStream_t s);
void launch_dgemm_f64_nt(const double *A, int64_t lda, const double *B,
                         int64_t ldb, double *C, int64_t ldc, int M, int64_t N,
                         int K, hipStream_t s);
void launch_dgemm_f64_nt_tril(const double *A, int64_t lda, const double *B,
                              int64_t ldb, double *C, int64_t ldc, int M,
                              int64_t N, int K, int v, int r0off,
                              int64_t c0off, int Px, int Py, int pi, int pj,
                              hipStream_t s);
void launch_init_matrix_spd(double *A, int Ml, int Nl, int v, int Px, int Py,
                            int pi, int pj, int zero_layer, uint64_t seed,
                            int64_t Nglob, hipStream_t s);
void launch_dgemm_f64(const double *A, int64_t lda, const double *B,
                      int64_t ldb, double *C, int64_t ldc, int M, int64_t N,
                      int K, hipStream_t s,
                      int maxwg = 0);
void launch_pack_candidate(const double *A10, int64_t lda, const int *gri,
                           int f, int n_src, int n_out, int v, const int *idx,
                           double *cand, hipStream_t s);
void launch_row_move(const double *src, int64_t lds, double *dst, int64_t ldd,
                     const int *src_idx, const int *dst_idx, int n_rows,
                     int64_t cols, hipStream_t s);
void launch_extract_col0_int(const double *cand, int stride, int n, int *out,
                             hipStream_t s);
void launch_slab_pack(const double *X, int64_t ldx, int n, int nlayr, int Pz,
                      double *out, hipStream_t s);
```

Before: 21.15 TFLOP/s.

## Add single-rank direct path: out-of-place TRSM from A11, skip staging copies

For a 1x1x1 grid, adds a direct mode, on by default, that removes the A10/A01 staging buffers. Both triangular solves now read straight from A11 and write into the receive buffers through new out-of-place stripe TRSM kernels. The triangle packing is hoisted to once per step and double-buffered by step parity. Row pushes are sliced so only the lookahead columns are swapped early, and the already-dead leading block is skipped. This cuts redundant copies, the reduce/NCCL paths and the per-solve pack launches, at the cost of more intricate stream ordering and buffer aliasing.

```diff
diff --git a/conflux_amd/__init__.py b/conflux_amd/__init__.py
--- a/conflux_amd/__init__.py
+++ b/conflux_amd/__init__.py
@@ -63,6 +63,11 @@
         ctypes.c_int, ctypes.c_int, ctypes.c_int, ctypes.c_longlong,
         ctypes.c_longlong, ctypes.c_longlong, ctypes.c_void_p,
         ctypes.c_void_p]
+    lib.conflux_lu_debug_set_one_rank_direct.argtypes = [ctypes.c_int]
+    lib.conflux_lu_debug_trsm_oop.argtypes = [
+        ctypes.c_int, ctypes.c_int, ctypes.c_longlong, ctypes.c_longlong,
+        ctypes.c_longlong, ctypes.c_longlong, ctypes.c_longlong,
+        ctypes.c_void_p, ctypes.c_void_p, ctypes.c_void_p]
     lib.conflux_lu_debug_dgemm_bench.argtypes = [
         ctypes.c_int, ctypes.c_longlong, ctypes.c_int, ctypes.c_int,
         ctypes.POINTER(ctypes.c_double)]
diff --git a/conflux_amd/csrc/engine.cpp b/conflux_amd/csrc/engine.cpp
--- a/conflux_amd/csrc/engine.cpp
+++ b/conflux_amd/csrc/engine.cpp
@@ -110,6 +110,7 @@
     std::vector<RankState> rs;
     std::vector<int> pivotInds;
     unsigned epoch = 1;
+    int direct = 0;
     std::vector<EvPair> evs;
     size_t evs_used = 0;
     TimeCat cats[4];
@@ -380,10 +381,10 @@
     return g_trsm_stripe;
 }
 
-int stripe_ws(RankState &r, int v, int which, double **ws) {
+int stripe_ws(RankState &r, int v, int which, double **ws, int set = 0) {
     const int64_t n = conflux_trsm_stripe_ws_doubles(v);
-    if (!r.triws) HIPCHK(hipMalloc(&r.triws, 2 * n * 8));
-    *ws = r.triws + which * n;
+    if (!r.triws) HIPCHK(hipMalloc(&r.triws, 4 * n * 8));
+    *ws = r.triws + (2 * set + which) * n;
     return 0;
 }
 
@@ -407,6 +408,52 @@
     } else
         launch_trsm_left_mfma(r.A00, v, X, ldx, v, N, s);
     return 0;
+}
+
+enum { ORD_SOLVES = 1, ORD_PUSH = 2, ORD_DEAD = 4, ORD_ALL = 7 };
+int g_one_rank_direct = -1;
+int one_rank_direct_mode() {
+    if (g_one_rank_direct < 0) {
+        const char *e = getenv("CONFLUX_ONE_RANK_DIRECT");
+        g_one_rank_direct = e ? (atoi(e) & ORD_ALL) : ORD_ALL;
+    }
+    return g_one_rank_direct;
+}
+int one_rank_direct_bits(const Ctx &c) {
+    if (c.sim || c.world != 1 || c.Px != 1 || c.Py != 1 || c.Pz != 1) return 0;
+    int bits = one_rank_direct_mode();
+    if (!(trsm_stripe_mode() && conflux_trsm_stripe_fits(c.v)))
+        bits &= ~ORD_SOLVES;
+    return bits;
+}
+
+int pack_step_triangles(Ctx &c, RankState &r, int k) {
+    double *wsu, *wsl;
+    if (stripe_ws(r, c.v, 0, &wsu, k & 1) || stripe_ws(r, c.v, 1, &wsl, k & 1))
+        return CONFLUX_LU_EHIP;
+    launch_trsm_pack_tri(r.A00, c.v, c.v, 0, 0, wsu, c.stream);
+    launch_trsm_pack_tri(r.A00, c.v, c.v, 1, 0, wsl, c.stream);
+    return 0;
+}
+
+int trsm_right_direct(Ctx &c, RankState &r, int k, const double *Xs,
+                      int64_t lds, double *Xd, int64_t ldd, int64_t M) {
+    double *ws;
+    size_t slot;
+    if (stripe_ws(r, c.v, 0, &ws, k & 1) || ev_begin(c, 2, 0, &slot))
+        return CONFLUX_LU_EHIP;
+    launch_trsm_right_stripe_packed(ws, Xs, lds, Xd, ldd, c.v, M, c.stream);
+    return ev_end(c, slot);
+}
+
+int trsm_left_direct(Ctx &c, RankState &r, int k, const double *Xs,
+                     int64_t lds, double *Xd, int64_t ldd, int64_t N) {
+    double *ws;
+    size_t slot;
+    if (stripe_ws(r, c.v, 1, &ws, k & 1) || ev_begin(c, 2, 0, &slot))
+        return CONFLUX_LU_EHIP;
+    launch_trsm_left_stripe_packed(ws, Xs, lds, Xd, ldd, c.v, N, c.stream);
+    return ev_end(c, slot);
 }
 
 int trsm_right_upper(Ctx &c, RankState &r, double *X, int64_t ldx, int M) {
@@ -705,6 +752,7 @@
     c.evs_used = 0;
     for (auto &t : c.cats) t = TimeCat{};
     g_gap = GapStats{};
+    c.direct = one_rank_direct_bits(c);
 
     int rc = timed_region(c, elapsed_ms, [&]() -> int {
         StepPlan sp;
@@ -757,12 +805,14 @@
     const int kcol = k % Py, krow = k % Px;
     const int n_rounds = Px > 1 ? (int)std::ceil(std::log2((double)Px)) : 0;
 
+    const bool direct = c.direct & ORD_SOLVES;
+
     for (auto &r : c.rs) {
-        if (r.pj != kcol) continue;
+        if (r.pj != kcol || direct) continue;
         launch_copy2d(r.A11 + i64(r.fnp) * Nl + loff, Nl,
                       r.A10 + i64(r.fnp) * v, v, r.nact, v, c.stream);
     }
-    {
+    if (!direct) {
         std::vector<ReduceItem> items;
         for (auto &r : c.rs)
             if (r.pj == kcol && (r.pk == 0 || !c.sim))
@@ -778,7 +828,12 @@
     for (auto &r : c.rs) {
         if (r.pj != kcol || r.pk != 0) continue;
         const int n = r.nact;
-        launch_copy2d(r.A10 + i64(r.fnp) * v, v, r.panel, v, n, v, c.stream);
+        if (direct)
+            launch_copy2d(r.A11 + i64(r.fnp) * Nl + loff, Nl, r.panel, v, n, v,
+                          c.stream);
+        else
+            launch_copy2d(r.A10 + i64(r.fnp) * v, v, r.panel, v, n, v,
+                          c.stream);
         std::vector<int> ipiv;
         if (n > 0) {
             if (factor_panel(c, r, n, ipiv)) return CONFLUX_LU_EINTERNAL;
@@ -806,6 +861,7 @@
 
         if (n_rounds == 0) {
             launch_copy2d(r.panel, v, r.A00, v, std::min(v, n), v, c.stream);
+            if (direct && pack_step_triangles(c, r, k)) return CONFLUX_LU_EHIP;
             for (int i = 0; i < v; ++i)
                 sp.gpivots[i] = (perm[i] < n) ? r.gri[r.fnp + perm[i]] : 0;
             if (!c.sim && c.world > 1)
@@ -943,6 +999,39 @@
     GapClock::time_point gap_t0;
     if (gap_on) gap_t0 = GapClock::now();
 
+    static int split_env = -1;
+    if (split_env < 0) {
+        const char *se = getenv("CONFLUX_SPLIT_TRSM");
+        split_env = se ? atoi(se) : 1;
+    }
+    const bool split_trsm = !c.sim && c.trsm_stream && split_env;
+    static int slice_env = -1;
+    if (slice_env < 0) {
+        const char *se2 = getenv("CONFLUX_SLICE_TRSM");
+        slice_env = se2 ? atoi(se2) : 1;
+    }
+    const char *lk_slice = getenv("CONFLUX_LOOKAHEAD");
+    const bool slice_first =
+        split_trsm && slice_env && Pz == 1 && Px == 1 && look &&
+        c.panel_stream && (lk_slice ? atoi(lk_slice) != 0 : true);
+    const bool direct = c.direct & ORD_SOLVES;
+    const bool sliced = (c.direct & ORD_PUSH) && slice_first;
+    const int64_t dead = (c.direct & ORD_DEAD) ? v : 0;
+    const int64_t wfirst = sliced ? lnext + v - loff : wA01;
+    auto push_rows = [&](RankState &r, double *mat, int64_t ld, int64_t col0,
+                         int64_t cols, int f, int cnt, int n_early) -> int {
+        size_t slot;
+        if (ev_begin(c, 3, 0, &slot)) return CONFLUX_LU_EHIP;
+        launch_row_gather(mat + col0, ld, r.rowtmp, cols, r.d_idx, cnt, cols,
+                          c.stream);
+        launch_row_move(mat + col0, ld, mat + col0, ld, r.d_idx + v,
+                        r.d_idx + 2 * v, n_early, cols, c.stream);
+        launch_copy2d(r.rowtmp, cols, mat + i64(f) * ld + col0, ld, cnt, cols,
+                      c.stream);
+        return ev_end(c, slot);
+    };
+    int n_early0 = 0;
+
     for (auto &r : c.rs) {
         const auto &lr = sp.lrows[r.pi];
         const auto &ord = sp.order[r.pi];
@@ -986,20 +1075,16 @@
         if (cnt)
             HIPCHK(hipMemcpyAsync(r.d_idx, stage, size_t(4) * v * 4,
                                   hipMemcpyHostToDevice, c.stream));
-        auto push = [&](double *mat, int64_t ld, int64_t cols) -> int {
-            size_t slot;
-            if (ev_begin(c, 3, 0, &slot)) return CONFLUX_LU_EHIP;
-            launch_row_gather(mat, ld, r.rowtmp, cols, r.d_idx, cnt, cols,
-                              c.stream);
-            launch_row_move(mat, ld, mat, ld, r.d_idx + v, r.d_idx + 2 * v,
-                            n_early, cols, c.stream);
-            launch_copy2d(r.rowtmp, cols, mat + i64(f) * ld, ld, cnt, cols,
-                          c.stream);
-            return ev_end(c, slot);
+        auto push = [&](double *mat, int64_t ld, int64_t col0,
+                        int64_t cols) -> int {
+            return push_rows(r, mat, ld, col0, cols, f, cnt, n_early);
         };
-        if (push(r.A11, Nl, Nl)) return CONFLUX_LU_EHIP;
-        if (push(r.A10, v, v)) return CONFLUX_LU_EHIP;
-        if (c.store_factors && push(r.A10hist, Nl, Nl)) return CONFLUX_LU_EHIP;
+        n_early0 = n_early;
+        if (sliced ? push(r.A11, Nl, loff, wfirst) : push(r.A11, Nl, 0, Nl))
+            return CONFLUX_LU_EHIP;
+        if (!direct && push(r.A10, v, 0, v)) return CONFLUX_LU_EHIP;
+        if (c.store_factors && push(r.A10hist, Nl, 0, Nl))
+            return CONFLUX_LU_EHIP;
         {
             GapClock::time_point gri_t0;
             if (gap_on) gri_t0 = GapClock::now();
@@ -1023,8 +1108,9 @@
         }
         r.fnp += cnt;
         r.nact -= cnt;
-        launch_copy2d(r.A11 + i64(f) * Nl + loff, Nl, r.A01pack, wA01, cnt,
-                      wA01, c.stream);
+        if (!direct)
+            launch_copy2d(r.A11 + i64(f) * Nl + loff, Nl, r.A01pack, wA01, cnt,
+                          wfirst, c.stream);
     }
     {
         std::vector<ReduceItem> items;
@@ -1035,7 +1121,8 @@
         if (depth_reduce(c, c.comm, items)) return CONFLUX_LU_ECOMM;
     }
 
-    if (!c.sim) {
+    if (direct) {
+    } else if (!c.sim) {
         RankState &me = c.rs[0];
         if (me.pk == 0) {
             NCCLCHK(ncclGroupStart());
@@ -1065,7 +1152,7 @@
                                           sp.order[krow].data(), cnt_own * 4,
                                           hipMemcpyHostToDevice, c.stream));
                     launch_row_scatter(me.A01pack, wA01, me.A01, wA01,
-                                       me.d_idx + 3 * v, cnt_own, wA01,
+                                       me.d_idx + 3 * v, cnt_own, wfirst,
                                        c.stream);
                 }
                 int64_t off = 0;
@@ -1121,12 +1208,15 @@
                     RankState &me = c.rs[0];
                     if (src && src->grank == me.grank && dst &&
                         dst->grank == me.grank) {
-                        HIPCHK(hipMemcpyAsync(me.d_idx + 2 * v,
-                                              sp.order[pi].data(), cnt * 4,
-                                              hipMemcpyHostToDevice, c.stream));
+                        int *const d_ord = me.d_idx + (sliced ? 3 : 2) * v;
+                        if (!sliced)
+                            HIPCHK(hipMemcpyAsync(d_ord, sp.order[pi].data(),
+                                                  cnt * 4,
+                                                  hipMemcpyHostToDevice,
+                                                  c.stream));
                         launch_row_scatter(me.A10hist + i64(me.fnp - cnt) * Nl,
                                            Nl, me.Fres + i64(ltik) * v * Nl,
-                                           Nl, me.d_idx + 2 * v, cnt, histcols,
+                                           Nl, d_ord, cnt, histcols,
                                            c.stream);
                     } else if (src && src->grank == me.grank) {
                         launch_copy2d(me.A10hist + i64(me.fnp - cnt) * Nl, Nl,
@@ -1153,30 +1243,48 @@
         }
     }
 
-    static int split_env = -1;
-    if (split_env < 0) {
-        const char *se = getenv("CONFLUX_SPLIT_TRSM");
-        split_env = se ? atoi(se) : 1;
-    }
-    const bool split_trsm = !c.sim && c.trsm_stream && split_env;
-    static int slice_env = -1;
-    if (slice_env < 0) {
-        const char *se2 = getenv("CONFLUX_SLICE_TRSM");
-        slice_env = se2 ? atoi(se2) : 1;
-    }
-    const char *lk_slice = getenv("CONFLUX_LOOKAHEAD");
-    const bool slice_first =
-        split_trsm && slice_env && Pz == 1 && Px == 1 && look &&
-        c.panel_stream && (lk_slice ? atoi(lk_slice) != 0 : true);
     auto store_u = [&](RankState &r) {
         if (!c.store_factors) return;
         double *Frow = r.Fres + i64(k / Px) * v * Nl;
-        const int64_t ustart = i64(v) * (r.pj < kcol ? k / Py + 1 : k / Py);
-        if (Nl - ustart > 0)
+        const int64_t ustart =
+            i64(v) * (r.pj < kcol ? k / Py + 1 : k / Py) + dead;
+        if (Nl - ustart > 0 && direct)
+            launch_copy2d(r.A01Rcv + (ustart - loff), Nl, Frow + ustart, Nl, v,
+                          Nl - ustart, c.stream);
+        else if (Nl - ustart > 0)
             launch_copy2d(r.A01 + (ustart - loff), wA01, Frow + ustart, Nl, v,
                           Nl - ustart, c.stream);
         if (r.pj == kcol)
             launch_copy2d(r.A00, v, Frow + loff, Nl, v, v, c.stream);
+    };
+    auto solve_left = [&](RankState &r, int64_t c0, int64_t w) -> int {
+        if (w <= 0) return 0;
+        if (direct)
+            return trsm_left_direct(c, r, k,
+                                    r.A11 + i64(r.fnp - v) * Nl + loff + c0, Nl,
+                                    r.A01Rcv + c0, Nl, w);
+        return trsm_left_lower(c, r, r.A01 + c0, wA01, w);
+    };
+    auto solve_rest = [&](RankState &r) -> int {
+        const int64_t s0 = lnext - loff;
+        if (sliced) {
+            const int64_t wrest = Nl - (lnext + v);
+            if (wrest > 0 &&
+                push_rows(r, r.A11, Nl, lnext + v, wrest, r.fnp - v, v,
+                          n_early0))
+                return CONFLUX_LU_EHIP;
+            if (wrest > 0 && !direct) {
+                launch_copy2d(r.A11 + i64(r.fnp - v) * Nl + lnext + v, Nl,
+                              r.A01pack + wfirst, wA01, v, wrest, c.stream);
+                launch_row_scatter(r.A01pack + wfirst, wA01, r.A01 + wfirst,
+                                   wA01, r.d_idx + 3 * v, v, wrest, c.stream);
+            }
+        }
+        if (dead < s0 && solve_left(r, dead, s0 - dead))
+            return CONFLUX_LU_EINTERNAL;
+        if (solve_left(r, s0 + v, wA01 - s0 - v)) return CONFLUX_LU_EINTERNAL;
+        store_u(r);
+        return 0;
     };
     if (gap_on) {
         g_gap.to_trsm += gap_ms(gap_t0, GapClock::now());
@@ -1189,22 +1297,19 @@
         c.stream = c.trsm_stream;
         for (auto &r : c.rs) {
             if (r.pi != krow || r.pk != 0) continue;
-            if (slice_first) {
-                const int64_t s0 = lnext - loff;
-                if (trsm_left_lower(c, r, r.A01 + s0, wA01, v))
+            if (!slice_first) {
+                if (solve_left(r, dead, wA01 - dead))
                     return CONFLUX_LU_EINTERNAL;
-                HIPCHK(hipEventRecord(c.ev_t5a, c.stream));
-                if (s0 > 0 && trsm_left_lower(c, r, r.A01, wA01, s0))
-                    return CONFLUX_LU_EINTERNAL;
-                if (wA01 - s0 - v > 0 &&
-                    trsm_left_lower(c, r, r.A01 + s0 + v, wA01,
-                                    wA01 - s0 - v))
-                    return CONFLUX_LU_EINTERNAL;
-            } else if (trsm_left_lower(c, r, r.A01, wA01, wA01))
-                return CONFLUX_LU_EINTERNAL;
-            store_u(r);
-        }
-        HIPCHK(hipEventRecord(c.ev_t5, c.stream));
+                store_u(r);
+                continue;
+            }
+            const int64_t s0 = lnext - loff;
+            if (solve_left(r, s0, v)) return CONFLUX_LU_EINTERNAL;
+            HIPCHK(hipEventRecord(c.ev_t5a, c.stream));
+            if (!sliced)
+                if (int rc = solve_rest(r)) return rc;
+        }
+        if (!sliced) HIPCHK(hipEventRecord(c.ev_t5, c.stream));
         c.stream = saved;
     }
 
@@ -1212,6 +1317,18 @@
         nanscan(c, "A11.postpush", k, r.A11, i64(c.Ml) * Nl);
     for (auto &r : c.rs) {
         if (r.pj != kcol || r.pk != 0) continue;
+        if (direct) {
+            nanscan(c, "A00", k, r.A00, i64(v) * v);
+            if (r.nact > 0 &&
+                trsm_right_direct(c, r, k, r.A11 + i64(r.fnp) * Nl + loff, Nl,
+                                  r.A10Rcv, c.nlayr, r.nact))
+                return CONFLUX_LU_EINTERNAL;
+            if (c.store_factors)
+                launch_copy2d(r.A10Rcv, c.nlayr,
+                              r.A10hist + i64(r.fnp) * Nl + loff, Nl, r.nact, v,
+                              c.stream);
+            continue;
+        }
         nanscan(c, "A10.pre", k, r.A10 + i64(r.fnp) * v, i64(r.nact) * v);
         nanscan(c, "A00", k, r.A00, i64(v) * v);
         if (trsm_right_upper(c, r, r.A10 + i64(r.fnp) * v, v, r.nact))
@@ -1222,15 +1339,15 @@
                           r.A10hist + i64(r.fnp) * Nl + loff, Nl, r.nact, v,
                           c.stream);
     }
-    if (int rc = spread_col_slabs(
-            c, kcol, [](const RankState &r) { return r.fnp; }))
-        return rc;
+    if (!direct)
+        if (int rc = spread_col_slabs(
+                c, kcol, [](const RankState &r) { return r.fnp; }))
+            return rc;
 
     if (!split_trsm) {
         for (auto &r : c.rs) {
             if (r.pi != krow || r.pk != 0) continue;
-            if (trsm_left_lower(c, r, r.A01, wA01, wA01))
-                return CONFLUX_LU_EINTERNAL;
+            if (solve_left(r, dead, wA01 - dead)) return CONFLUX_LU_EINTERNAL;
             store_u(r);
         }
     } else if (!slice_first) {
@@ -1245,10 +1362,12 @@
         else if (slice_first) {
             HIPCHK(hipStreamWaitEvent(c.stream, c.ev_t5a, 0));
             const int64_t s0 = lnext - loff;
-            launch_copy2d(r.A01 + s0, wA01, r.A01Rcv + s0, Nl, c.nlayr, v,
-                          c.stream);
-        } else
-            launch_copy2d(r.A01, wA01, r.A01Rcv, Nl, c.nlayr, wA01, c.stream);
+            if (!direct)
+                launch_copy2d(r.A01 + s0, wA01, r.A01Rcv + s0, Nl, c.nlayr, v,
+                              c.stream);
+        } else if (!direct)
+            launch_copy2d(r.A01 + dead, wA01, r.A01Rcv + dead, Nl, c.nlayr,
+                          wA01 - dead, c.stream);
     } else if (int rc = spread_row_panel(
                    c, krow, [&](int) { return wA01; },
                    [](int) { return int64_t(0); }))
@@ -1313,21 +1432,33 @@
     }
     if (slice_first) {
         RankState &r = c.rs[0];
+        if (sliced) {
+            hipStream_t saved = c.stream;
+            HIPCHK(hipStreamWaitEvent(c.trsm_stream, c.ev_pc, 0));
+            c.stream = c.trsm_stream;
+            const int rc = solve_rest(r);
+            if (!rc) HIPCHK(hipEventRecord(c.ev_t5, c.stream));
+            c.stream = saved;
+            if (rc) return rc;
+        }
         HIPCHK(hipStreamWaitEvent(c.stream, c.ev_t5, 0));
         const int64_t s0 = lnext - loff;
-        if (s0 > 0)
-            launch_copy2d(r.A01, wA01, r.A01Rcv, Nl, c.nlayr, s0, c.stream);
-        if (wA01 - s0 - v > 0)
+        if (!direct && s0 > dead)
+            launch_copy2d(r.A01 + dead, wA01, r.A01Rcv + dead, Nl, c.nlayr,
+                          s0 - dead, c.stream);
+        if (!direct && wA01 - s0 - v > 0)
             launch_copy2d(r.A01 + s0 + v, wA01, r.A01Rcv + s0 + v, Nl,
                           c.nlayr, wA01 - s0 - v, c.stream);
     }
     for (auto &r : c.rs) {
         if (look && r.pj == ncol) {
-            if (gemm_piece(r, loff, lnext - loff, gcap)) return CONFLUX_LU_EHIP;
+            if (gemm_piece(r, loff + dead, lnext - loff - dead, gcap))
+                return CONFLUX_LU_EHIP;
             if (gemm_piece(r, lnext + v, Nl - (lnext + v), gcap))
                 return CONFLUX_LU_EHIP;
         } else {
-            if (gemm_piece(r, loff, wA01, gcap)) return CONFLUX_LU_EHIP;
+            if (gemm_piece(r, loff + dead, wA01 - dead, gcap))
+                return CONFLUX_LU_EHIP;
         }
     }
     if (look) {
@@ -3012,6 +3143,59 @@
     return rc;
 }
 
+int conflux_lu_debug_set_one_rank_direct(int mode) {
+    const int prev = one_rank_direct_mode();
+    g_one_rank_direct = mode & ORD_ALL;
+    return prev;
+}
+
+int conflux_lu_debug_trsm_oop(int side_right, int v, int64_t n, int64_t lds,
+                              int64_t soff, int64_t ldd, int64_t doff,
+                              const double *T, double *Xs, double *Xd) {
+    const int64_t w = side_right ? i64(v) : n;
+    if (v <= 0 || n <= 0 || !T || !Xs || soff < 0 || lds < soff + w ||
+        (Xd && (doff < 0 || ldd < doff + w)) || n > INT32_MAX ||
+        !conflux_trsm_stripe_fits(v))
+        return CONFLUX_LU_EARG;
+    const int64_t rows = side_right ? n : i64(v);
+    double *dT = nullptr, *dS = nullptr, *dD = nullptr, *ws = nullptr;
+    auto cleanup = [&]() {
+        for (double *p : {dT, dS, dD, ws})
+            if (p) (void)hipFree(p);
+    };
+    hipError_t e = hipMalloc(&dT, i64(v) * v * 8);
+    if (e == hipSuccess) e = hipMalloc(&dS, rows * lds * 8);
+    if (e == hipSuccess && Xd) e = hipMalloc(&dD, rows * ldd * 8);
+    if (e == hipSuccess)
+        e = hipMalloc(&ws, conflux_trsm_stripe_ws_doubles(v) * 8);
+    if (e == hipSuccess)
+        e = hipMemcpy(dT, T, i64(v) * v * 8, hipMemcpyHostToDevice);
+    if (e == hipSuccess)
+        e = hipMemcpy(dS, Xs, rows * lds * 8, hipMemcpyHostToDevice);
+    if (e == hipSuccess && Xd)
+        e = hipMemcpy(dD, Xd, rows * ldd * 8, hipMemcpyHostToDevice);
+    if (e == hipSuccess) {
+        double *dst = Xd ? dD + doff : dS + soff;
+        const int64_t ld2 = Xd ? ldd : lds;
+        launch_trsm_pack_tri(dT, v, v, side_right ? 0 : 1, 0, ws, nullptr);
+        if (side_right)
+            launch_trsm_right_stripe_packed(ws, dS + soff, lds, dst, ld2, v, n,
+                                            nullptr);
+        else
+            launch_trsm_left_stripe_packed(ws, dS + soff, lds, dst, ld2, v, n,
+                                           nullptr);
+        e = hipGetLastError();
+    }
+    if (e == hipSuccess) e = hipDeviceSynchronize();
+    if (e == hipSuccess)
+        e = hipMemcpy(Xs, dS, rows * lds * 8, hipMemcpyDeviceToHost);
+    if (e == hipSuccess && Xd)
+        e = hipMemcpy(Xd, dD, rows * ldd * 8, hipMemcpyDeviceToHost);
+    cleanup();
+    HIPCHK(e);
+    return CONFLUX_LU_OK;
+}
+
 int conflux_lu_debug_trsm_left(int upper, int unit, int v, int64_t N,
                                int64_t ldt, const double *T, double *X) {
     if (v <= 0 || N <= 0 || ldt < v || !T || !X) return CONFLUX_LU_EARG;
diff --git a/conflux_amd/csrc/kernels.hip b/conflux_amd/csrc/kernels.hip
--- a/conflux_amd/csrc/kernels.hip
+++ b/conflux_amd/csrc/kernels.hip
@@ -2374,8 +2374,8 @@
 }
 
 __global__ __launch_bounds__(256) void k_trsm_right_stripe(
-    const double *__restrict__ U, double *__restrict__ X, int64_t ldx, int v,
-    int64_t M) {
+    const double *__restrict__ U, const double *Xs, int64_t lds, double *Xd,
+    int64_t ldd, int v, int64_t M) {
     __shared__ double sX[TRS_MAXP][TRS_W][33];
     __shared__ double sU[2][32][33];
     const int tid = threadIdx.x;
@@ -2399,7 +2399,7 @@
     load_u_regs(0, 0);
     for (int i = tid; i < TRS_W * v; i += 256) {
         const int r = i / v, cc = i - r * v;
-        sX[cc >> 5][r][cc & 31] = r < rows ? X[(r0 + r) * ldx + cc] : 0.0;
+        sX[cc >> 5][r][cc & 31] = r < rows ? Xs[(r0 + r) * lds + cc] : 0.0;
     }
     write_u(0);
     __syncthreads();
@@ -2447,13 +2447,13 @@
     }
     for (int i = tid; i < rows * v; i += 256) {
         const int r = i / v, cc = i - r * v;
-        X[(r0 + r) * ldx + cc] = sX[cc >> 5][r][cc & 31];
+        Xd[(r0 + r) * ldd + cc] = sX[cc >> 5][r][cc & 31];
     }
 }
 
 __global__ __launch_bounds__(256) void k_trsm_left_stripe(
-    const double *__restrict__ L, double *__restrict__ X, int64_t ldx, int v,
-    int64_t N) {
+    const double *__restrict__ L, const double *Xs, int64_t lds, double *Xd,
+    int64_t ldd, int v, int64_t N) {
     __shared__ double sX[TRS_MAXP][32][TRS_W + 1];
     __shared__ double sL[2][32][33];
     const int tid = threadIdx.x;
@@ -2478,7 +2478,7 @@
     for (int i = tid; i < v * TRS_W; i += 256) {
         const int r = i >> 5, cc = i & (TRS_W - 1);
         sX[r >> 5][r & 31][cc] =
-            cc < cols ? X[(int64_t)r * ldx + c0 + cc] : 0.0;
+            cc < cols ? Xs[(int64_t)r * lds + c0 + cc] : 0.0;
     }
     write_l(0);
     __syncthreads();
@@ -2525,7 +2525,7 @@
     }
     for (int i = tid; i < v * TRS_W; i += 256) {
         const int r = i >> 5, cc = i & (TRS_W - 1);
-        if (cc < cols) X[(int64_t)r * ldx + c0 + cc] = sX[r >> 5][r & 31][cc];
+        if (cc < cols) Xd[(int64_t)r * ldd + c0 + cc] = sX[r >> 5][r & 31][cc];
     }
 }
 
@@ -2537,28 +2537,46 @@
 int64_t conflux_trsm_stripe_ws_doubles(int v) {
     const int64_t np = v / 32;
     return np * (np + 1) / 2 * 1024;
+}
+
+void launch_trsm_pack_tri(const double *T, int64_t ldt, int v, int swap,
+                          int tr, double *ws, hipStream_t s) {
+    if (v <= 0) return;
+    const int nblk = (int)(conflux_trsm_stripe_ws_doubles(v) / 1024);
+    hipLaunchKernelGGL(k_trsm_pack_tri, dim3(nblk), dim3(256), 0, s, T, ldt, ws,
+                       swap, tr);
+}
+
+void launch_trsm_right_stripe_packed(const double *ws, const double *Xs,
+                                     int64_t lds, double *Xd, int64_t ldd,
+                                     int v, int64_t M, hipStream_t s) {
+    if (M <= 0 || v <= 0) return;
+    hipLaunchKernelGGL(k_trsm_right_stripe, dim3(cdiv64(M, TRS_W)), dim3(256),
+                       0, s, ws, Xs, lds, Xd, ldd, v, M);
+}
+
+void launch_trsm_left_stripe_packed(const double *ws, const double *Xs,
+                                    int64_t lds, double *Xd, int64_t ldd,
+                                    int v, int64_t N, hipStream_t s) {
+    if (N <= 0 || v <= 0) return;
+    hipLaunchKernelGGL(k_trsm_left_stripe, dim3(cdiv64(N, TRS_W)), dim3(256),
+                       0, s, ws, Xs, lds, Xd, ldd, v, N);
 }
 
 void launch_trsm_right_stripe(const double *U, int64_t ldu, double *X,
                               int64_t ldx, int v, int64_t M, int trans,
                               double *ws, hipStream_t s) {
     if (M <= 0 || v <= 0) return;
-    const int nblk = (int)(conflux_trsm_stripe_ws_doubles(v) / 1024);
-    hipLaunchKernelGGL(k_trsm_pack_tri, dim3(nblk), dim3(256), 0, s, U, ldu, ws,
-                       trans ? 1 : 0, trans ? 1 : 0);
-    hipLaunchKernelGGL(k_trsm_right_stripe, dim3(cdiv64(M, TRS_W)), dim3(256),
-                       0, s, ws, X, ldx, v, M);
+    launch_trsm_pack_tri(U, ldu, v, trans ? 1 : 0, trans ? 1 : 0, ws, s);
+    launch_trsm_right_stripe_packed(ws, X, ldx, X, ldx, v, M, s);
 }
 
 void launch_trsm_left_stripe(const double *L, int64_t ldl, double *X,
                              int64_t ldx, int v, int64_t N, double *ws,
                              hipStream_t s) {
     if (N <= 0 || v <= 0) return;
-    const int nblk = (int)(conflux_trsm_stripe_ws_doubles(v) / 1024);
-    hipLaunchKernelGGL(k_trsm_pack_tri, dim3(nblk), dim3(256), 0, s, L, ldl, ws,
-                       1, 0);
-    hipLaunchKernelGGL(k_trsm_left_stripe, dim3(cdiv64(N, TRS_W)), dim3(256),
-                       0, s, ws, X, ldx, v, N);
+    launch_trsm_pack_tri(L, ldl, v, 1, 0, ws, s);
+    launch_trsm_left_stripe_packed(ws, X, ldx, X, ldx, v, N, s);
 }
 
 void launch_trsm_right_mfma(const double *U, int64_t ldu, double *X,
diff --git a/conflux_amd/csrc/kernels.hpp b/conflux_amd/csrc/kernels.hpp
--- a/conflux_amd/csrc/kernels.hpp
+++ b/conflux_amd/csrc/kernels.hpp
@@ -68,6 +68,14 @@
 void launch_trsm_left_stripe(const double *L, int64_t ldl, double *X,
                              int64_t ldx, int v, int64_t N, double *ws,
                              hipStream_t s);
+void launch_trsm_pack_tri(const double *T, int64_t ldt, int v, int swap,
+                          int tr, double *ws, hipStream_t s);
+void launch_trsm_right_stripe_packed(const double *ws, const double *Xs,
+                                     int64_t lds, double *Xd, int64_t ldd,
+                                     int v, int64_t M, hipStream_t s);
+void launch_trsm_left_stripe_packed(const double *ws, const double *Xs,
+                                    int64_t lds, double *Xd, int64_t ldd,
+                                    int v, int64_t N, hipStream_t s);
 void launch_trsm_left_tri_mfma(const double *T, int64_t ldt, double *X,
                                int64_t ldx, int v, int64_t N, int upper,
                                int unit, hipStream_t s);
```

After: 21.98 TFLOP/s, median of 6. 3.9% higher.
